# av-savchenko/HSE_FaceRec_tf

Measured on AMD Instinct MI355X. Metric: faces/sec embedding-extract (MobileNet-192, bs=256), higher is better.
Workload: dtype f32

## Files before the change

### hse_facerec_tf_amd/_lib.py

```python
from __future__ import annotations

import ctypes
import os
from ctypes import POINTER, c_char_p, c_float, c_int, c_longlong, c_size_t, c_void_p

_HERE = os.path.dirname(os.path.abspath(__file__))
LIB_PATH = os.path.join(_HERE, os.environ.get("HSEFR_LIB", "libhsefr.so"))

OK, ERR_INVALID, ERR_UNSUPPORTED, ERR_HIP, ERR_NOMEM, ERR_SHAPE = 0, -1, -2, -3, -4, -5

_lib = None

_fp = c_void_p
SIGNATURES = {
    "hsefr_version": (c_int, []),
    "hsefr_last_error_string": (c_char_p, []),
    "hsefr_engine_set_graph_batch": (c_int, [c_void_p, c_int]),
    "hsefr_engine_graph_launches": (c_longlong, [c_void_p]),
    "hsefr_engine_create": (c_int, [c_void_p, c_size_t, c_int, POINTER(c_void_p)]),
    "hsefr_plan_validate": (c_int, [c_void_p, c_size_t]),
    "hsefr_plan_describe": (c_int, [c_void_p, c_size_t, c_int, c_char_p, c_size_t]),
    "hsefr_engine_workspace_bytes": (c_size_t, [c_void_p]),
    "hsefr_engine_max_batch": (c_int, [c_void_p]),
    "hsefr_engine_forward": (c_int, [c_void_p, _fp, c_int, _fp, _fp, _fp, c_void_p]),
    "hsefr_engine_buffer": (c_void_p, [c_void_p, c_int]),
    "hsefr_engine_copy_buffer": (c_int, [c_void_p, c_int, _fp, c_size_t, c_void_p]),
    "hsefr_engine_set_profiling": (c_int, [c_void_p, c_int]),
    "hsefr_engine_profiled_calls": (c_longlong, [c_void_p]),
    "hsefr_engine_op_times_ms": (c_int, [c_void_p, c_int, POINTER(c_float), c_int]),
    "hsefr_engine_destroy": (c_int, [c_void_p]),
    "hsefr_conv_c3_bias_act": (c_int, [_fp, _fp, _fp, _fp] + [c_int] * 12 + [c_void_p]),
    "hsefr_dwconv3x3_bn_relu6": (c_int, [_fp, _fp, _fp, _fp, _fp] + [c_int] * 10 + [c_void_p]),
    "hsefr_dwconv3x3_bn_relu6_split": (c_int, [_fp, _fp, _fp, _fp, _fp] + [c_int] * 11 + [c_void_p]),
    "hsefr_pwconv1x1_presplit_gap": (c_int, [_fp, c_void_p, _fp, _fp, _fp, c_longlong, c_int, c_int, c_int, c_int, c_void_p]),
    "hsefr_pwconv1x1_presplit_dw": (c_int, [_fp, c_void_p, _fp, _fp, _fp, _fp, c_longlong] + [c_int] * 7 + [c_void_p]),
    "hsefr_pwconv1x1_presplit": (c_int, [_fp, c_void_p, _fp, _fp, _fp, c_longlong, c_int, c_int, c_int, c_void_p]),
    "hsefr_pwconv1x1_bias_relu6": (c_int, [_fp, _fp, _fp, _fp, c_longlong, c_int, c_int, c_int, c_void_p]),
    "hsefr_stem2_fused": (c_int, [_fp] * 6 + [c_void_p] + [_fp] * 6 + [c_int] * 13 + [c_void_p]),
    "hsefr_stem3_fused": (c_int, [_fp, c_void_p] + [_fp] * 5 + [c_void_p] + [_fp] * 7 + [c_int] * 14 + [c_void_p]),
    "hsefr_stem4_fused": (c_int, [_fp, c_int, c_void_p] + [_fp] * 5 + [c_void_p] + [_fp] * 7 + [c_int] * 6 + [c_void_p]),
    "hsefr_stem5_stream": (c_int, [_fp, c_int, c_void_p] + [_fp] * 5 + [c_void_p] + [_fp] * 7 + [c_int] * 6 + [c_void_p]),
    "hsefr_engine_accepts_u8": (c_int, [c_void_p]),
    "hsefr_engine_forward_u8": (c_int, [c_void_p, _fp, c_int, _fp, _fp, _fp, c_void_p]),
    "hsefr_engine_input_overflow": (c_int, [c_void_p, POINTER(c_int), c_void_p]),
    "hsefr_engine_input_overflow_async": (c_int, [c_void_p, POINTER(c_int), c_void_p]),
    "hsefr_dwpw_f16split": (c_int, [_fp, _fp, _fp, _fp, c_void_p, _fp, _fp, _fp] + [c_int] * 12 + [c_void_p]),
    "hsefr_pwconv1x1_f16split": (c_int, [_fp, c_void_p, _fp, _fp, _fp, c_longlong, c_int, c_int, c_int, c_int, c_void_p]),
    "hsefr_dwpw_fused": (c_int, [_fp] * 7 + [c_int] * 10 + [c_void_p]),
    "hsefr_gap": (c_int, [_fp, _fp, c_int, c_int, c_int, c_void_p]),
    "hsefr_dense": (c_int, [_fp, _fp, _fp, _fp, c_int, c_int, c_int, c_int, c_void_p]),
    "hsefr_softmax": (c_int, [_fp, _fp, c_int, c_int, c_void_p]),
    "hsefr_heads_fused": (c_int, [_fp] * 11 + [c_int] * 3 + [c_void_p]),
    "hsefr_conv_bf16": (c_int, [_fp, _fp, _fp, _fp, _fp, _fp] + [c_int] * 13 + [c_void_p]),
    "hsefr_conv1x1_proj_bf16": (c_int, [_fp] * 9 + [c_int] * 10 + [c_void_p]),
    "hsefr_conv1x1_sres_bf16": (c_int, [_fp] * 6 + [c_int] * 9 + [c_void_p]),
    "hsefr_conv1x1_pair_bf16": (c_int, [_fp] * 14 + [c_longlong] + [c_int] * 6 + [c_void_p]),
    "hsefr_conv1x1_pair_sub2_bf16": (c_int, [_fp] * 14 + [c_int] * 9 + [c_void_p]),
    "hsefr_stem7x7_bf16": (c_int, [_fp, _fp, _fp, _fp, _fp] + [c_int] * 6 + [c_void_p]),
    "hsefr_stem7x7_pool_bf16": (c_int, [_fp, c_void_p, _fp, _fp, c_void_p] + [c_int] * 7 + [c_void_p]),
    "hsefr_maxpool3x3s2_bf16": (c_int, [_fp, _fp] + [c_int] * 8 + [c_void_p]),
    "hsefr_gap_bf16": (c_int, [_fp, _fp, c_int, c_int, c_int, c_void_p]),
    "hsefr_preprocess_pil_u8": (c_int, [_fp, _fp, _fp] + [c_int] * 5 + [_fp, _fp, _fp, c_int, _fp, _fp, _fp, c_int, c_int,
                                        POINTER(ctypes.c_double), c_void_p]),
    "hsefr_preprocess_cv_u8": (c_int, [_fp, _fp] + [c_int] * 5 + [_fp] * 6 + [c_int, POINTER(ctypes.c_double), c_void_p]),
    "hsefr_l2_normalize": (c_int, [_fp, _fp, c_int, c_int, c_void_p]),
    "hsefr_conv2d_direct": (c_int, [_fp] * 5 + [c_int] * 12 + [c_void_p]),
    "hsefr_conv2d_f32": (c_int, [_fp] * 6 + [c_int] * 13 + [c_void_p]),
    "hsefr_conv2d_f32_mfma": (c_int, [_fp] * 6 + [c_int] * 13 + [c_void_p]),
    "hsefr_maxpool_f32": (c_int, [_fp, _fp] + [c_int] * 10 + [c_void_p]),
    "hsefr_mtcnn_pyramid_level": (c_int, [_fp, _fp, c_int, c_int, c_int, c_int, c_void_p]),
    "hsefr_mtcnn_post_capacity": (c_int, []),
    "hsefr_mtcnn_stage1_level": (c_int, [_fp, _fp, c_int, c_int, ctypes.c_double, ctypes.c_float, _fp, _fp, c_void_p]),
    "hsefr_mtcnn_stage1_finish": (c_int, [_fp, _fp, _fp, _fp, c_int, c_int, c_void_p]),
    "hsefr_mtcnn_stage_finish": (c_int, [c_int, _fp, c_int, _fp, _fp, _fp, ctypes.c_float, _fp, _fp, _fp, _fp, c_int, c_int, c_void_p]),
    "hsefr_mtcnn_nms": (c_int, [_fp, c_int, ctypes.c_double, c_int, _fp, _fp, c_void_p]),
    "hsefr_mtcnn_crops": (c_int, [_fp, _fp, _fp, c_int, c_int, c_int, c_int, c_void_p]),
    "hsefr_pairwise_dist": (c_int, [_fp, _fp, c_int, c_int, c_int, _fp, c_void_p]),
    "hsefr_single_linkage": (c_int, [_fp, c_int, c_int, _fp, _fp, _fp, _fp, _fp, _fp, c_void_p]),
    "hsefr_hier_linkage": (c_int, [_fp, c_int, c_int, _fp, _fp, _fp, c_int, _fp, _fp, _fp, _fp, c_void_p]),
    "hsefr_dbscan": (c_int, [_fp, c_int, c_int, _fp, _fp, _fp, ctypes.c_double, c_int, _fp, _fp, c_void_p]),
    "hsefr_rank_order": (c_int, [_fp, c_int, c_int, _fp, _fp, _fp, ctypes.c_double, ctypes.c_double, _fp, POINTER(c_int), c_void_p]),
    "hsefr_rank_order_sweep": (c_int, [_fp, c_int, c_int, _fp, _fp, _fp, POINTER(ctypes.c_double), c_int, _fp, POINTER(c_int), c_void_p]),
    "hsefr_flat_cuts": (c_int, [_fp, _fp, c_int, _fp, c_int, _fp, c_void_p]),
    "hsefr_partition_scores": (c_int, [_fp, _fp, c_int, c_int, _fp, _fp, c_void_p]),
    "hsefr_nn1": (c_int, [_fp, _fp, c_int, c_int, c_int, _fp, _fp, c_void_p]),
    "hsefr_knn": (c_int, [_fp, _fp, c_int, c_int, c_int, c_int, _fp, _fp, _fp, _fp, c_void_p]),
    "hsefr_nn1_fallbacks": (c_longlong, []),
    "hsefr_pca_fit": (c_int, [_fp, c_int, c_int, c_int, c_int, _fp, _fp, _fp, _fp, c_void_p]),
    "hsefr_pca_transform": (c_int, [_fp, c_int, c_int, c_int, _fp, _fp, _fp, c_int, c_void_p]),
    "hsefr_linear_svm_fit": (c_int, [_fp, c_int, c_int, _fp, c_int, ctypes.c_double, ctypes.c_double, c_int, _fp, _fp, _fp, c_void_p]),
    "hsefr_linear_svm_decision": (c_int, [_fp, c_int, c_int, _fp, _fp, c_int, _fp, c_void_p]),
    "hsefr_linear_svm_predict": (c_int, [_fp, c_int, c_int, _fp, c_void_p]),
    "hsefr_rbf_svm_gamma_scale": (c_int, [_fp, c_int, c_int, c_int, _fp, c_void_p]),
    "hsefr_rbf_svm_fit": (c_int, [_fp, c_int, c_int, _fp, c_int, ctypes.c_double, ctypes.c_double, ctypes.c_double, c_int, _fp, _fp, _fp,
                                  c_void_p]),
    "hsefr_rbf_svm_decision": (c_int, [_fp, c_int, _fp, c_int, c_int, _fp, c_int, ctypes.c_double, _fp, _fp, _fp, c_void_p]),
    "hsefr_rbf_svm_predict": (c_int, [_fp, c_int, _fp, c_int, c_int, _fp, c_int, ctypes.c_double, _fp, _fp, _fp, _fp, c_void_p]),
}

DEV_SIGNATURES = {
    "hsefr_debug_set": (c_int, [c_char_p, c_int]),
    "hsefr_debug_read_stamps": (c_int, [c_int, c_void_p, ctypes.c_size_t]),
    "hsefr_debug_clock_probe": (c_int, [_fp, c_int, c_int, c_void_p]),
    "hsefr_debug_copy": (c_int, [_fp, _fp, c_size_t, c_void_p]),
    "hsefr_stem_fused": (c_int, [_fp] * 6 + [c_void_p, _fp, _fp, _fp] + [c_int] * 9 + [c_void_p]),
}


class HsefrError(RuntimeError):
    pass


def lib() -> ctypes.CDLL:
    global _lib
    if _lib is None:
        import torch
        if not os.path.exists(LIB_PATH):
            raise ImportError("%s is missing: build it with `python -c 'import __graft_entry__ as g; g.build()'` "
                              "(hipcc --offload-arch=gfx950). There is no CPU fallback." % LIB_PATH)
        L = ctypes.CDLL(LIB_PATH)
        for name, (res, args) in SIGNATURES.items():
            fn = getattr(L, name)
            fn.restype = res
            fn.argtypes = args
        for name, (res, args) in DEV_SIGNATURES.items():
            if hasattr(L, name):
                fn = getattr(L, name)
                fn.restype = res
                fn.argtypes = args
# ... 75 lines not shown
```

### hse_facerec_tf_amd/csrc/common.h

```cpp
#pragma once
#include <hip/hip_runtime.h>
#include <stdarg.h>
#include <stdio.h>

#include "../../include/hsefr.h"
#ifdef HSEFR_DEV
#include "hsefr_dev.h"
#endif

namespace hsefr {

void set_error(const char* fmt, ...);

#define HSEFR_HIP_CHECK(expr)                                                          \
    do {                                                                               \
        hipError_t _e = (expr);                                                        \
        if (_e != hipSuccess) {                                                        \
            ::hsefr::set_error("%s failed: %s (%s:%d)", #expr, hipGetErrorString(_e),  \
                               __FILE__, __LINE__);                                    \
            return HSEFR_ERR_HIP;                                                      \
        }                                                                              \
    } while (0)

#define HSEFR_REQUIRE(cond, code, ...)     \
// ... 167 lines not shown
bool conv3x3_win_bf16_supported(long long n, int h, int w, int c, int cout);
int launch_conv3x3_win_bf16(const void* x, const void* wt, const float* scale, const float* shift, const void* res, void* y, int n, int h,
                            int w, int c, int cout, int act, hipStream_t s);
bool conv3x3_w2_forced();
bool conv3x3_w2_bf16_supported(long long n, int h, int w, int c, int cout);
bool conv3x3_w2_bf16_preferred(int h, int w, int cout);
int launch_conv3x3_w2_bf16(const void* x, const void* wt, const float* scale, const float* shift, const void* res, void* y, int n, int h,
                           int w, int c, int cout, int act, hipStream_t s);
bool conv1x1_w4_forced();
bool conv1x1_w4_bf16_supported(long long n, int h, int w, int c, int oh, int ow, int cout, int stride);
bool conv1x1_w4_bf16_preferred(long long pixels, int c, int cout, bool has_res);
bool conv1x1_w4_proj_preferred(long long pixels, int c, int c2, int cout);
int launch_conv1x1_w4_proj_bf16(const void* x, const void* wt, const float* scale, const float* shift, const void* x2, const void* wt2,
                                const float* scale2, const float* shift2, void* y, int n, int oh, int ow, int c, int cout, int c2, int stride2,
                                int h2, int w2, int act, hipStream_t s);
int launch_conv1x1_w4_bf16(const void* x, const void* wt, const float* scale, const float* shift, const void* res, void* y, int n, int h,
                           int w, int c, int oh, int ow, int cout, int stride, int act, hipStream_t s);
bool conv1x1_pair_bf16_shape_supported(int c, int cout1, int cout2, int c2);
bool conv1x1_pair_bf16_supported(long long pixels, int c, int cout1, int cout2, int c2);
int launch_conv1x1_pair_bf16(const void* x, const void* w1, const float* scale1, const float* shift1, const void* res, const void* x2,
                             const void* wp, const float* scale_p, const float* shift_p, void* y1, const void* w2, const float* scale2,
                             const float* shift2, void* y2, long long pixels, int c, int cout1, int cout2, int c2, int act1, int act2,
                             hipStream_t s, int y1_stride = 1, int h = 0, int w = 0);
bool conv_dma_forced();
bool conv_dma_bf16_supported(long long n, int h, int w, int c, int oh, int ow, int cout, int kh, int kw);
int launch_conv_dma_bf16(const void* x, const void* wt, const float* scale, const float* shift, const void* res, void* y, int n, int h,
                         int w, int c, int oh, int ow, int cout, int kh, int kw, int stride, int pad_t, int pad_l, int act, hipStream_t s);
int launch_stem7x7_pool_bf16(const float* x, const void* wt, const float* scale, const float* shift, void* y, int n, int h, int w,
                             int ph, int pw, int pool_pad_t, int pool_pad_l, hipStream_t s, const void* wfrag = nullptr);
bool stem7s_stream_supported(long long n, int h, int w, int ph, int pw);
int launch_stem7s_stream(const float* x, const void* wt, const float* scale, const float* shift, void* y, int n, int h, int w, int ph, int pw,
                         int pool_pad_t, int pool_pad_l, hipStream_t s, const void* wfrag = nullptr);
constexpr size_t STEM7S_WFRAG_BYTES = 4 * 7 * 64 * 16;
int stem7s_reorder_weights(const void* wt, void* wfrag, hipStream_t s);
int launch_maxpool3x3s2_bf16(const void* x, void* y, int n, int h, int w, int c, int oh, int ow, int pad_t, int pad_l,
                             hipStream_t s);
int launch_gap_bf16(const void* x, float* y, int n, int hw, int c, hipStream_t s);

int launch_pil_resize(const unsigned char* in, unsigned char* tmp, float* out, int n, int H, int W, int oh, int ow, const int* xmin,
                      const int* xcnt, const int* xcoef, int xk, const int* ymin, const int* ycnt, const int* ycoef, int yk,
                      int mode, const double* mean, hipStream_t s);
int launch_cv_resize(const unsigned char* in, float* out, int n, int H, int W, int oh, int ow, const int* x0, const int* x1,
                     const int* wx1, const int* y0, const int* y1, const int* wy1, int mode, const double* mean, hipStream_t s);

int launch_area_level(const unsigned char* src, float* dst, int sh, int sw, int dh, int dw, hipStream_t s);
int launch_area_crops(const unsigned char* src, const int* boxes, float* dst, int sh, int sw, int n, int size, hipStream_t s);
int launch_pairwise_dist(const float* x, const float* y, int n, int m, int d, float* out, hipStream_t s);
struct DistSource {
    const float* x;
    int n, d;
    const float* born;
    const float* year;
    const double* dense;
};
int launch_single_linkage(const DistSource& src, int* edge_a, int* edge_b, double* edge_h, hipStream_t s);
int launch_dbscan(const DistSource& src, double eps, int min_samples, int* labels, unsigned char* core, hipStream_t s);
int launch_rank_order(const DistSource& src, const double* thresholds, int pairs, int* labels, int* iterations, hipStream_t s);
int launch_hier_linkage(const DistSource& src, int method, int* merge_a, int* merge_b, double* merge_h, int* merge_round, hipStream_t s);
int launch_flat_cuts(const int* order, const double* gaps, int n, const double* thresholds, int rows, int* labels, hipStream_t s);
int launch_partition_scores(const int* y_true, const int* labels, int n, int rows, long long* counts, double* stats, hipStream_t s);

bool dwpw_fused_supported(int c, int cout, int stride, int act_dw, int act_pw);
int launch_dwpw_fused(const float* x, const float* wd, const float* dscale, const float* dshift, const float* wp_t,
                      const float* pshift, float* y, int n, int h, int w, int c, int stride, int pad_t, int pad_l, int oh,
                      int ow, int cout, int act_dw, int act_pw, hipStream_t s);

int launch_conv2d_direct(const float* x, const float* w, const float* bias, const float* alpha, float* y, int n, int h, int wd, int c,
                         int oh, int ow, int cout, int kh, int kw, int stride, int pad_t, int pad_l, hipStream_t s);
int launch_conv_f32_mfma(const float* x, const float* w, const float* scale, const float* shift, const float* res, float* y, int n, int h,
                         int wd, int c, int oh, int ow, int cout, int kh, int kw, int stride, int pad_t, int pad_l, int act, hipStream_t s,
                         int res_stride = 0, int res_h = 0, int res_w = 0);
bool conv_f32_mfma_supported(int c, int cout);
int launch_conv2d_f32(const float* x, const float* w, const float* scale, const float* shift, const float* res, float* y, int n, int h,
                      int wd, int c, int oh, int ow, int cout, int kh, int kw, int stride, int pad_t, int pad_l, int act, hipStream_t s);
int launch_maxpool_f32(const float* x, float* y, int n, int h, int w, int c, int oh, int ow, int k, int stride, int pad_t, int pad_l,
                       hipStream_t s);

int launch_dwpw_f16s(const float* x, const float* wd, const float* dscale, const float* dshift, const void* wsplit,
                     const float* descale, const float* pshift, float* y, int n, int h, int w, int c, int stride, int pad_t,
                     int pad_l, int oh, int ow, int cout, int a_log2, int act, hipStream_t s);
bool dwpw_f16s_supported(int c, int cout, int stride);
bool dwpw_s2_covered(int c, int cout, int stride);
bool dwpw_s2_off();
int launch_stem_fused(const float* x, const float* cw, const float* cshift, const float* wd, const float* dscale,
                      const float* dshift, const void* wsplit, const float* descale, const float* pshift, float* y, int n,
                      int h, int w, int cpad_t, int cpad_l, int oh, int ow, int a_log2, int act, hipStream_t s);
int launch_stem2_fused(const float* x, const float* cw, const float* cshift, const float* wd1, const float* d1scale,
                       const float* d1shift, const void* wsplit, const float* descale, const float* pshift, const float* wd2,
                       const float* d2scale, const float* d2shift, float* y, int n, int h, int w, int cpad_t, int cpad_l,
                       int h1, int w1, int pad_t2, int pad_l2, int oh2, int ow2, int a_log2, int act, hipStream_t s);
int launch_stem3_fused(const float* x, const void* cw_split, const float* cdescale, const float* cshift, const float* wd1,
                       const float* d1scale, const float* d1shift, const void* wsplit, const float* descale, const float* pshift,
                       const float* wd2, const float* d2scale, const float* d2shift, float* y, int* overflow, int n, int h, int w,
                       int cpad_t, int cpad_l, int h1, int w1, int pad_t2, int pad_l2, int oh2, int ow2, int in_log2, int a_log2,
                       int act, hipStream_t s);
bool stem3_fused_supported(int cin, int c1, int c2, int conv_stride, int dw1_stride, int dw2_stride, int kh, int kw);
int launch_stem4_fused(const void* x, int x_is_u8, const void* cw4, const float* cdescale, const float* cshift, const float* wd1,
                       const float* d1scale, const float* d1shift, const void* wsplit, const float* descale, const float* pshift,
                       const float* wd2, const float* d2scale, const float* d2shift, float* y, int* overflow, int n, int h, int w,
                       int in_log2, int a_log2, int act, hipStream_t s);
bool stem4_fused_supported(int cin, int c1, int c2, int conv_stride, int dw1_stride, int dw2_stride, int kh, int kw, int h, int w);
int launch_stem5_stream(const void* x, int x_is_u8, const void* cw4, const float* cdescale, const float* cshift, const float* wd1,
                        const float* d1scale, const float* d1shift, const void* wsplit, const float* descale, const float* pshift,
                        const float* wd2, const float* d2scale, const float* d2shift, float* y, int* overflow, int n, int h, int w,
                        int in_log2, int a_log2, int act, hipStream_t s);
bool stem5_stream_supported(int cin, int c1, int c2, int conv_stride, int dw1_stride, int dw2_stride, int kh, int kw, int h, int w);
bool stem2_fused_supported(int cin, int c1, int c2, int conv_stride, int dw1_stride, int dw2_stride, int kh, int kw);
bool stem_fused_supported(int cin, int cmid, int cout, int conv_stride, int dw_stride, int kh, int kw);
int read_pws_stamps(void* host_out, size_t bytes);
int read_stem_stamps(void* host_out, size_t bytes);
#ifdef HSEFR_STEM_STAMPS
unsigned long long* stamp_buffer(hipStream_t s);
#define STEM_STAMP(i) do { const unsigned long long _t = __builtin_amdgcn_s_memtime(); st[i] += _t - tprev; tprev = _t; } while (0)
#define STEM_STAMP_DECL unsigned long long st[8] = {0, 0, 0, 0, 0, 0, 0, 0}; unsigned long long tprev = __builtin_amdgcn_s_memtime(); \
    const unsigned long long tstart = tprev; unsigned npatch = 0
#define STEM_STAMP_COUNT ++npatch
#define STEM_STAMP_FLUSH(buf, lane, wave) do { if ((lane) == 0 && (buf) && blockIdx.x < 512) { unsigned long long* o = (buf) + (blockIdx.x * 4 + (wave)) * 10; \
    for (int i_ = 0; i_ < 8; ++i_) o[i_] = st[i_]; o[8] = __builtin_amdgcn_s_memtime() - tstart; o[9] = npatch; } } while (0)
#else
#define STEM_STAMP(i) do { } while (0)
#define STEM_STAMP_DECL do { } while (0)
#define STEM_STAMP_COUNT do { } while (0)
#define STEM_STAMP_FLUSH(buf, lane, wave) do { } while (0)
#endif
#ifdef HSEFR_DEV
int read_c11_stamps(void* host_out, size_t bytes);
int read_w4_stamps(void* host_out, size_t bytes);
int read_s7_stamps(void* host_out, size_t bytes);
int read_w2_stamps(void* host_out, size_t bytes);
int read_w3_stamps(void* host_out, size_t bytes);
int read_cd_stamps(void* host_out, size_t bytes);
int read_ps_stamps(void* host_out, size_t bytes);
int launch_clock_probe(unsigned long long* out, int blocks, int iters, hipStream_t s);
int launch_copy(const void* src, void* dst, size_t bytes, hipStream_t s);
#endif

}
```

### hse_facerec_tf_amd/csrc/engine.hip

```cpp
#include <math.h>
#include <string.h>

#include <cxxabi.h>
#include <dlfcn.h>
#include <elf.h>

#include <map>
#include <new>
#include <string>
#include <vector>

#include "common.h"

namespace hsefr {

static thread_local char g_err[512] = "";

void set_error(const char* fmt, ...) {
    va_list ap;
    va_start(ap, fmt);
    vsnprintf(g_err, sizeof(g_err), fmt, ap);
    va_end(ap);
}

// ... 185 lines not shown
                break;
            case HSEFR_OP_PWCONV_PS_GAP:
                HSEFR_REQUIRE(pwconv_ps_gap_supported(0, o.cin, o.cout, o.h * o.w) && o.oh == 1 && o.ow == 1, HSEFR_ERR_UNSUPPORTED,
                              "plan op %u: fused pointwise + global pool on a %dx%d map not covered (33 .. 288 pixels)", i, o.h, o.w);
                if (!need(o.w_off, ci * co * 4, "split rows") || !need(o.scale_off, co * 4, "descale") || !need(o.shift_off, co * 4, "shift"))
                    return HSEFR_ERR_INVALID;
                HSEFR_REQUIRE(o.aux > 0 && o.aux <= 24, HSEFR_ERR_INVALID, "plan op %u: a_log2 out of range (reserved %d)", i, o.aux);
                break;
            case HSEFR_OP_PWCONV_PS_DW:
                HSEFR_REQUIRE(pwconv_ps_dw_supported(0, o.cin, o.cout, o.w, o.h * o.w, o.stride) && o.oh * o.stride == o.h && o.ow * o.stride == o.w &&
                                  (o.stride == 1 ? (o.pad_t == 1 && o.pad_l == 1) : (o.pad_t == 0 && o.pad_l == 0)),
                              HSEFR_ERR_UNSUPPORTED, "plan op %u: fused pointwise + depthwise (stride %d) on a %dx%d map not covered", i, o.stride, o.h, o.w);
                if (!need(o.w_off, ci * co * 4, "split rows") || !need(o.scale_off, co * 4, "descale") || !need(o.shift_off, co * 4, "shift") ||
                    !need(o.w2_off, 11 * co * 4, "depthwise constants"))
                    return HSEFR_ERR_INVALID;
                {
                    const PsDwAux a = ps_dw_aux(o.aux);
                    HSEFR_REQUIRE(a.a_log2 > 0 && a.a_log2 <= 24 && a.out_log2 >= 1 && a.out_log2 <= 12,
                                  HSEFR_ERR_INVALID, "plan op %u: a_log2 / out_log2 out of range (reserved %d)", i, o.aux);
                }
                break;
            case HSEFR_OP_PWCONV_PS:
                HSEFR_REQUIRE(pwconv_ps_supported(0, o.cin, o.cout), HSEFR_ERR_UNSUPPORTED,
                              "plan op %u: pre-split pointwise cin=%d cout=%d not covered", i, o.cin, o.cout);
                [[fallthrough]];
            case HSEFR_OP_PWCONV_F16S:
                if (!need(o.w_off, ci * co * 4, "split rows") || !need(o.scale_off, co * 4, "descale") || !need(o.shift_off, co * 4, "shift"))
                    return HSEFR_ERR_INVALID;
                HSEFR_REQUIRE(o.w_off != HSEFR_NO_OFFSET && o.scale_off != HSEFR_NO_OFFSET && o.shift_off != HSEFR_NO_OFFSET &&
                                  o.aux > 0 && o.aux <= 24,
                              HSEFR_ERR_INVALID, "plan op %u: split-f16 pointwise needs split rows, descale, shift and a_log2 in (0, 24]", i);
                break;
            case HSEFR_OP_STEM3_F16S: {
                const StemAux a = stem_aux(o.aux);
                HSEFR_REQUIRE(stem3_fused_supported(o.cin, 32, o.cout, o.stride, 1, 2, o.kh, stem_kw(o.kw).k) && a.a_log2 > 0 && a.a_log2 <= 12 &&
                                  a.in_log2 >= -8 && a.in_log2 <= 14 &&
                                  o.w_off != HSEFR_NO_OFFSET && o.w2_off != HSEFR_NO_OFFSET && o.shift2_off != HSEFR_NO_OFFSET &&
                                  o.w_off + HSEFR_STEM_PACK_STEM3_END * 4 <= h.blob_bytes && o.w2_off + 64 * 128 <= h.blob_bytes &&
                                  o.shift2_off + 128 * 4 <= h.blob_bytes && o.in_buf == HSEFR_BUF_INPUT,
                              HSEFR_ERR_UNSUPPORTED, "plan op %u: bounded fused stem cin=%d cout=%d stride=%d not covered", i, o.cin, o.cout, o.stride);
                break;
            }
            case HSEFR_OP_STEM2_F16S:
                HSEFR_REQUIRE(stem2_fused_supported(o.cin, 32, o.cout, o.stride, 1, 2, o.kh, stem_kw(o.kw).k) && o.aux > 0 && o.aux <= 12 &&
                                  o.w_off != HSEFR_NO_OFFSET && o.w2_off != HSEFR_NO_OFFSET && o.shift2_off != HSEFR_NO_OFFSET &&
                                  o.w_off + HSEFR_STEM_PACK_STEM2_END * 4 <= h.blob_bytes && o.in_buf == HSEFR_BUF_INPUT,
                              HSEFR_ERR_UNSUPPORTED, "plan op %u: fused stem+dw2 cin=%d cout=%d stride=%d not covered", i, o.cin, o.cout, o.stride);
                break;
            case HSEFR_OP_STEM_F16S:
#ifndef HSEFR_DEV
                set_error("plan op %u: HSEFR_OP_STEM_F16S (round 1's fused stem) runs on development builds of the library only", i);
                return HSEFR_ERR_UNSUPPORTED;
#else
                HSEFR_REQUIRE(stem_fused_supported(o.cin, 32, o.cout, o.stride, 1, o.kh, o.kw) && o.aux > 0 && o.aux <= 12 &&
                                  o.w_off != HSEFR_NO_OFFSET && o.w2_off != HSEFR_NO_OFFSET && o.shift2_off != HSEFR_NO_OFFSET &&
                                  o.w_off + HSEFR_STEM_PACK_DW2 * 4 <= h.blob_bytes && o.in_buf == HSEFR_BUF_INPUT,
                              HSEFR_ERR_UNSUPPORTED, "plan op %u: fused stem cin=%d cout=%d stride=%d not covered", i, o.cin, o.cout, o.stride);
                break;
#endif
            case HSEFR_OP_DWPW_F16S:
                if (!need(o.w_off, 9 * ci * 4, "depthwise kernel") || !need(o.scale_off, ci * 4, "scale") || !need(o.shift_off, ci * 4, "shift") ||
                    !need(o.w2_off, ci * co * 4, "split rows") || !need(o.shift2_off, 2 * co * 4, "descale | shift"))
                    return HSEFR_ERR_INVALID;
                HSEFR_REQUIRE(dwpw_f16s_supported(o.cin, o.cout, o.stride) && o.aux > 0 && o.aux <= 12 &&
                                  o.w_off != HSEFR_NO_OFFSET && o.scale_off != HSEFR_NO_OFFSET && o.shift_off != HSEFR_NO_OFFSET &&
                                  o.w2_off != HSEFR_NO_OFFSET && o.shift2_off != HSEFR_NO_OFFSET,
                              HSEFR_ERR_UNSUPPORTED, "plan op %u: split-f16 fused block cin=%d cout=%d stride=%d a_log2=%d not covered",
                              i, o.cin, o.cout, o.stride, o.aux);
                break;
            case HSEFR_OP_DWPW_F32:
                if (!need(o.w_off, 9 * ci * 4, "depthwise kernel") || !need(o.scale_off, ci * 4, "scale") || !need(o.shift_off, ci * 4, "shift") ||
                    !need(o.w2_off, ci * co * 4, "pointwise kernel") || !need(o.shift2_off, co * 4, "pointwise shift"))
                    return HSEFR_ERR_INVALID;
                HSEFR_REQUIRE(dwpw_fused_supported(o.cin, o.cout, o.stride, HSEFR_ACT_RELU6, (int)o.act), HSEFR_ERR_UNSUPPORTED,
                              "plan op %u: fused depthwise-pointwise block cin=%d cout=%d not covered", i, o.cin, o.cout);
                break;
            default:
                set_error("plan op %u: unknown kind %u", i, o.kind);
                return HSEFR_ERR_UNSUPPORTED;
        }
    }
    for (uint32_t i = 0; i < h.n_ops; ++i) {
        const hsefr_plan_op& o = ops[i];
        HSEFR_REQUIRE((o.flags & ~(HSEFR_OPF_PAIR_NEXT | HSEFR_OPF_HEADS | HSEFR_OPF_OUT_SUB2 | HSEFR_OPF_DWPW_NEXT)) == 0, HSEFR_ERR_INVALID,
                      "plan op %u: unknown flags 0x%x", i, o.flags);
        HSEFR_REQUIRE(!(o.flags & HSEFR_OPF_OUT_SUB2) || (o.flags & HSEFR_OPF_PAIR_NEXT), HSEFR_ERR_INVALID, "plan op %u: OUT_SUB2 without PAIR_NEXT", i);
        if (o.flags & HSEFR_OPF_PAIR_NEXT) {
            HSEFR_REQUIRE(i + 1 < h.n_ops, HSEFR_ERR_INVALID, "plan op %u: PAIR_NEXT on the last op", i);
            const hsefr_plan_op& b = ops[i + 1];
            const bool proj = o.w2_off != HSEFR_NO_OFFSET;
            const Geometry g = geometry(o.aux);
            const int c2 = proj ? g.c2 : 0;
            const bool sub2 = (o.flags & HSEFR_OPF_OUT_SUB2) != 0;
            HSEFR_REQUIRE(o.kind == HSEFR_OP_CONV_BF16 && b.kind == HSEFR_OP_CONV_BF16 && o.kh == 1 && o.kw == 1 && o.stride == 1 && o.pad_t == 0 &&
                              o.pad_l == 0 && (sub2 ? (o.oh == (o.h + 1) / 2 && o.ow == (o.w + 1) / 2 && o.h > 1 && o.w > 1) : (o.oh == o.h && o.ow == o.w)) &&
                              b.kh == 1 && b.kw == 1 && b.stride == 1 && b.pad_t == 0 && b.pad_l == 0 &&
                              b.h == o.h && b.w == o.w && b.oh == b.h && b.ow == b.w && b.cin == o.cout && b.in_buf == o.out_buf &&
                              b.res_buf == HSEFR_BUF_NONE && b.w2_off == HSEFR_NO_OFFSET && b.flags == 0 && o.res_buf >= 0 &&
                              (!proj || (g.stride2 == 1 && g.h2 == o.h && g.w2 == o.w)),
                          HSEFR_ERR_INVALID, "plan op %u: PAIR_NEXT needs two 1x1 stride-1 bf16 convolutions at the same pixels, the first with a residual "
                          "or a same-pixel projected shortcut, the second reading the first", i);
            HSEFR_REQUIRE(b.out_buf != o.in_buf && b.out_buf != o.res_buf && b.out_buf != o.out_buf, HSEFR_ERR_INVALID,
                          "plan op %u: PAIR_NEXT: the second output (buffer %d) aliases an operand of the first", i, b.out_buf);
            HSEFR_REQUIRE(conv1x1_pair_bf16_shape_supported(o.cin, o.cout, b.cout, c2), HSEFR_ERR_UNSUPPORTED,
                          "plan op %u: PAIR_NEXT %d -> %d -> %d (projection from %d) not covered", i, o.cin, o.cout, b.cout, c2);
        }
        if (o.flags & HSEFR_OPF_DWPW_NEXT) {
            HSEFR_REQUIRE(o.flags == HSEFR_OPF_DWPW_NEXT && i + 1 < h.n_ops, HSEFR_ERR_INVALID, "plan op %u: DWPW_NEXT on the last op or beside another flag", i);
            const hsefr_plan_op& b = ops[i + 1];
            HSEFR_REQUIRE(o.kind == HSEFR_OP_DWCONV3X3 && o.stride == 2 && o.act == HSEFR_ACT_RELU6 && o.aux == 0 && o.cout == o.cin &&
                              b.kind == HSEFR_OP_PWCONV_F16S && b.in_buf == o.out_buf && b.flags == 0 && b.h == o.oh && b.w == o.ow && b.oh == b.h &&
                              b.ow == b.w && b.cin == o.cin && b.aux > 0 && b.aux <= 12,
                          HSEFR_ERR_INVALID, "plan op %u: DWPW_NEXT needs a stride-2 depthwise 3x3 with ReLU6 and fp32 output, and behind it a split-f16 "
                          "pointwise op without flags that reads it at the same pixels (a_log2 in [1, 12])", i);
            HSEFR_REQUIRE(dwpw_s2_covered(o.cin, b.cout, o.stride), HSEFR_ERR_INVALID, "plan op %u: DWPW_NEXT %d -> %d channels not covered (128 -> 256)", i,
                          o.cin, b.cout);
            HSEFR_REQUIRE(b.out_buf != o.out_buf, HSEFR_ERR_INVALID, "plan op %u: DWPW_NEXT: the second output (buffer %d) aliases the depthwise tensor", i,
                          b.out_buf);
            HSEFR_REQUIRE(b.out_buf != o.in_buf || (uint64_t)bufs[o.in_buf].elems_per_image * bufs[o.in_buf].elem_bytes ==
                                                       (uint64_t)bufs[o.out_buf].elems_per_image * bufs[o.out_buf].elem_bytes,
                          HSEFR_ERR_INVALID, "plan op %u: DWPW_NEXT: buffers %d and %d exchange roles and must have one size", i, o.in_buf, o.out_buf);
            for (uint32_t k = i + 2; k < h.n_ops; ++k) {
                HSEFR_REQUIRE(ops[k].in_buf != o.out_buf && ops[k].res_buf != o.out_buf, HSEFR_ERR_INVALID,
                              "plan op %u: DWPW_NEXT: op %u also reads the depthwise tensor (buffer %d)", i, k, o.out_buf);
                if (ops[k].out_buf == o.out_buf) break;
            }
            for (int sl = 0; sl < HSEFR_N_OUTPUT_SLOTS; ++sl)
                HSEFR_REQUIRE(h.out_buffer[sl] != o.out_buf && (b.out_buf != o.in_buf || h.out_buffer[sl] != o.in_buf), HSEFR_ERR_INVALID,
                              "plan op %u: DWPW_NEXT: the depthwise tensor (or the buffer it exchanges roles with) is output slot %d", i, sl);
        }
        if (o.flags & HSEFR_OPF_HEADS) {
            HSEFR_REQUIRE(i + 3 < h.n_ops, HSEFR_ERR_INVALID, "plan op %u: HEADS needs three ops behind it", i);
            const hsefr_plan_op &a = ops[i + 1], &sm = ops[i + 2], &g = ops[i + 3];
            HSEFR_REQUIRE(o.kind == HSEFR_OP_DENSE && o.act == HSEFR_ACT_RELU && o.cout == 256 && o.cin > 0 && o.cin % 256 == 0 && o.cin <= 2048 &&
                              o.shift_off != HSEFR_NO_OFFSET && a.kind == HSEFR_OP_DENSE && a.act == HSEFR_ACT_NONE && a.cin == 256 && a.cout >= 1 &&
                              a.cout <= 128 && a.in_buf == o.out_buf && a.shift_off != HSEFR_NO_OFFSET && sm.kind == HSEFR_OP_SOFTMAX &&
                              sm.in_buf == a.out_buf && sm.cout == a.cout && g.kind == HSEFR_OP_DENSE && g.act == HSEFR_ACT_SIGMOID && g.cin == 256 &&
                              g.cout == 1 && g.in_buf == o.out_buf && g.shift_off != HSEFR_NO_OFFSET && a.flags == 0 && sm.flags == 0 && g.flags == 0,
                          HSEFR_ERR_INVALID, "plan op %u: HEADS needs DENSE k -> 256 + ReLU, DENSE 256 -> a (<= 128) + bias, SOFTMAX, DENSE 256 -> 1 + sigmoid", i);
            const int outs[4] = {o.out_buf, a.out_buf, sm.out_buf, g.out_buf};
            for (int x = 0; x < 4; ++x) {
                HSEFR_REQUIRE(outs[x] != o.in_buf, HSEFR_ERR_INVALID, "plan op %u: HEADS: an output aliases the pooled features", i);
                for (int y = x + 1; y < 4; ++y)
                    HSEFR_REQUIRE(outs[x] != outs[y], HSEFR_ERR_INVALID, "plan op %u: HEADS: two of the four tensors share buffer %d", i, outs[x]);
            }
        }
    }
    for (int s = 0; s < HSEFR_N_OUTPUT_SLOTS; ++s) {
        HSEFR_REQUIRE(h.out_buffer[s] == HSEFR_BUF_NONE || (h.out_buffer[s] >= 0 && h.out_buffer[s] < (int)h.n_buffers),
                      HSEFR_ERR_INVALID, "plan: output slot %d names buffer %d", s, h.out_buffer[s]);
        if (h.out_buffer[s] == HSEFR_BUF_NONE) continue;
        const int b = h.out_buffer[s];
        uint32_t producers = 0;
        for (uint32_t i = 0; i < h.n_ops; ++i) producers += (ops[i].out_buf == b);
        HSEFR_REQUIRE(producers == 1, HSEFR_ERR_INVALID, "plan: output slot %d: buffer %d has %u producing ops (must be exactly 1)", s, b,
                      producers);
        HSEFR_REQUIRE((uint64_t)bufs[b].elems_per_image * bufs[b].elem_bytes == (uint64_t)h.out_elems[s] * 4, HSEFR_ERR_INVALID,
                      "plan: output slot %d: buffer %d holds %llu x %u bytes per image, the slot declares %u fp32 elements", s, b,
                      (unsigned long long)bufs[b].elems_per_image, (unsigned)bufs[b].elem_bytes, h.out_elems[s]);
    }
    return HSEFR_OK;
}

namespace hsefr {
#ifdef HSEFR_STEM_STAMPS
static unsigned long long* g_stamp_buf = nullptr;
unsigned long long* stamp_buffer(hipStream_t s) {
    if (!g_stamp_buf && hipMalloc((void**)&g_stamp_buf, 512 * 4 * 10 * 8) != hipSuccess) return nullptr;
    (void)hipMemsetAsync(g_stamp_buf, 0, 512 * 4 * 10 * 8, s);
    return g_stamp_buf;
}
int read_stem_stamps(void* host_out, size_t bytes) {
    HSEFR_REQUIRE(g_stamp_buf && bytes <= 512 * 4 * 10 * 8, HSEFR_ERR_INVALID, "read_stem_stamps: nothing recorded / too many bytes");
    HSEFR_HIP_CHECK(hipMemcpy(host_out, g_stamp_buf, bytes, hipMemcpyDeviceToHost));
    return HSEFR_OK;
}
#else
int read_stem_stamps(void* host_out, size_t bytes) {
    (void)host_out; (void)bytes;
    set_error("read_stem_stamps: library built without -DHSEFR_STEM_STAMPS");
    return HSEFR_ERR_UNSUPPORTED;
}
#endif
static thread_local std::string* g_route_sink = nullptr;
bool route_probe() { return g_route_sink != nullptr; }
static const std::map<uintptr_t, std::string>& stub_names() {
    static const std::map<uintptr_t, std::string> table = [] {
        std::map<uintptr_t, std::string> m;
        Dl_info info;
        if (!dladdr(reinterpret_cast<const void*>(&stub_names), &info) || !info.dli_fname) return m;
        FILE* f = fopen(info.dli_fname, "rb");
        if (!f) return m;
        std::vector<unsigned char> img;
        fseek(f, 0, SEEK_END);
        const long sz = ftell(f);
        fseek(f, 0, SEEK_SET);
        if (sz > 0) { img.resize((size_t)sz); if (fread(img.data(), 1, img.size(), f) != img.size()) img.clear(); }
        fclose(f);
        if (img.size() < sizeof(Elf64_Ehdr)) return m;
        const Elf64_Ehdr* eh = reinterpret_cast<const Elf64_Ehdr*>(img.data());
        if (memcmp(eh->e_ident, ELFMAG, SELFMAG) != 0 || eh->e_shentsize != sizeof(Elf64_Shdr) ||
            eh->e_shoff + (uint64_t)eh->e_shnum * sizeof(Elf64_Shdr) > img.size()) return m;
        const Elf64_Shdr* sh = reinterpret_cast<const Elf64_Shdr*>(img.data() + eh->e_shoff);
        for (int i = 0; i < eh->e_shnum; ++i) {
            if (sh[i].sh_type != SHT_SYMTAB || sh[i].sh_link >= eh->e_shnum) continue;
            const Elf64_Shdr& st = sh[sh[i].sh_link];
            if (sh[i].sh_offset + sh[i].sh_size > img.size() || st.sh_offset + st.sh_size > img.size()) continue;
            const Elf64_Sym* sym = reinterpret_cast<const Elf64_Sym*>(img.data() + sh[i].sh_offset);
            const char* str = reinterpret_cast<const char*>(img.data() + st.sh_offset);
            for (size_t k = 0; k < sh[i].sh_size / sizeof(Elf64_Sym); ++k) {
                if (ELF64_ST_TYPE(sym[k].st_info) != STT_OBJECT || sym[k].st_name >= st.sh_size) continue;
                const char* nm = str + sym[k].st_name;
// ... 182 lines not shown

int hsefr_engine_copy_buffer(hsefr_engine* e, int buffer, void* d_dst, size_t bytes, hsefr_stream_t stream) {
    HSEFR_REQUIRE(e && d_dst, HSEFR_ERR_INVALID, "copy_buffer: null argument");
    HSEFR_REQUIRE(buffer >= 0 && buffer < (int)e->d_bufs.size(), HSEFR_ERR_INVALID, "copy_buffer: buffer %d", buffer);
    const size_t cap = (size_t)e->bufs[buffer].elems_per_image * e->bufs[buffer].elem_bytes * e->max_batch;
    HSEFR_REQUIRE(bytes <= cap, HSEFR_ERR_SHAPE, "copy_buffer: %zu bytes exceed buffer %d (%zu)", bytes, buffer, cap);
    HSEFR_HIP_CHECK(hipMemcpyAsync(d_dst, e->d_bufs[buffer], bytes, hipMemcpyDeviceToDevice, (hipStream_t)stream));
    return HSEFR_OK;
}

int hsefr_engine_set_profiling(hsefr_engine* e, int depth) {
    HSEFR_REQUIRE(e && depth >= 0, HSEFR_ERR_INVALID, "set_profiling: bad argument");
    for (auto ev : e->events) (void)hipEventDestroy(ev);
    e->events.clear();
    e->prof_depth = 0;
    e->prof_calls = 0;
    if (depth > 0) {
        e->events.resize((size_t)depth * (e->ops.size() + 1));
        for (auto& ev : e->events) HSEFR_HIP_CHECK(hipEventCreate(&ev));
        e->prof_depth = depth;
    }
    return HSEFR_OK;
}

long long hsefr_engine_profiled_calls(const hsefr_engine* e) { return e ? e->prof_calls : 0; }

int hsefr_engine_op_times_ms(hsefr_engine* e, int slot, float* ms, int n_ops) {
    HSEFR_REQUIRE(e && ms, HSEFR_ERR_INVALID, "op_times: null argument");
    HSEFR_REQUIRE(e->prof_depth > 0 && slot >= 0 && slot < e->prof_depth && slot < e->prof_calls, HSEFR_ERR_INVALID,
                  "op_times: slot %d has no profiled forward (depth %d, calls %lld)", slot, e->prof_depth, e->prof_calls);
    HSEFR_REQUIRE(n_ops == (int)e->ops.size(), HSEFR_ERR_INVALID, "op_times: expected %zu ops", e->ops.size());
    hipEvent_t* ev = e->events.data() + (size_t)slot * (e->ops.size() + 1);
    HSEFR_HIP_CHECK(hipEventSynchronize(ev[n_ops]));
    for (int i = 0; i < n_ops; ++i) HSEFR_HIP_CHECK(hipEventElapsedTime(&ms[i], ev[i], ev[i + 1]));
    return HSEFR_OK;
}

struct Operands {
    const void *w, *w2;
    const float *scale, *shift, *shift2;
};
static Operands operands(const hsefr_engine* e, const hsefr_plan_op& o) {
    return {blob_ptr(e, o.w_off), blob_ptr(e, o.w2_off), (const float*)blob_ptr(e, o.scale_off), (const float*)blob_ptr(e, o.shift_off),
            (const float*)blob_ptr(e, o.shift2_off)};
}

static int launch_op(hsefr_engine* e, size_t i, std::vector<void*>& tab, const void* d_input, int n, const std::vector<char>& needed, hipStream_t s,
                     bool input_u8, bool every_tensor, size_t& covered) {
    const hsefr_plan_op& o = e->ops[i];
    const Operands p = operands(e, o);
    const void* in = buf_ptr(tab, o.in_buf, d_input);
    void* out = buf_ptr(tab, o.out_buf, d_input);
    const long long pixels = (long long)n * o.h * o.w;
    covered = 0;
    const bool sub2 = (o.flags & HSEFR_OPF_OUT_SUB2) != 0;
    const Geometry g = geometry(o.aux);
    const bool proj = o.w2_off != HSEFR_NO_OFFSET;
    const int c2 = proj ? g.c2 : 0;
    const bool pair_ok = (o.flags & HSEFR_OPF_PAIR_NEXT) && needed[i + 1] &&
                         conv1x1_pair_bf16_supported(pixels, o.cin, o.cout, e->ops[i + 1].cout, c2);
    HSEFR_REQUIRE(!sub2 || pair_ok, HSEFR_ERR_UNSUPPORTED, "forward: op %zu stores its output at every second pixel (OUT_SUB2) and cannot run without the pair launch", i);
    if (pair_ok) {
        const hsefr_plan_op& b = e->ops[i + 1];
        const Operands pb = operands(e, b);
        covered = 1;
        return launch_conv1x1_pair_bf16(in, p.w, p.scale, p.shift, proj ? nullptr : tab[o.res_buf], proj ? tab[o.res_buf] : nullptr, proj ? p.w2 : nullptr,
                                        proj ? p.shift2 : nullptr, proj ? p.shift2 + o.cout : nullptr, out, pb.w, pb.scale, pb.shift, tab[b.out_buf],
                                        pixels, o.cin, o.cout, b.cout, c2, o.act, b.act, s, sub2 ? 2 : 1, o.h, o.w);
    }
    if ((o.flags & HSEFR_OPF_HEADS) && !g_heads_off && needed[i + 1] && needed[i + 2] && needed[i + 3]) {
        const hsefr_plan_op &a = e->ops[i + 1], &sm = e->ops[i + 2], &gd = e->ops[i + 3];
        const Operands pa = operands(e, a), pg = operands(e, gd);
        covered = 3;
        return launch_heads_fused((const float*)in, (const float*)p.w, p.shift, (const float*)pa.w, pa.shift, (const float*)pg.w, pg.shift, (float*)out,
                                  (float*)tab[a.out_buf], (float*)tab[sm.out_buf], (float*)tab[gd.out_buf], n, o.cin, a.cout, s);
    }
    if ((o.flags & HSEFR_OPF_DWPW_NEXT) && !every_tensor && !dwpw_s2_off() && needed[i + 1]) {
        const hsefr_plan_op& b = e->ops[i + 1];
        const Operands pb = operands(e, b);
        if (b.out_buf == o.in_buf) std::swap(tab[o.in_buf], tab[o.out_buf]);
        covered = 1;
        return launch_dwpw_f16s((const float*)in, (const float*)p.w, p.scale, p.shift, pb.w, pb.scale, pb.shift, (float*)tab[b.out_buf], n, o.h, o.w,
                                o.cin, o.stride, o.pad_t, o.pad_l, o.oh, o.ow, b.cout, b.aux, b.act, s);
    }
    const void* res = o.res_buf >= 0 ? tab[o.res_buf] : nullptr;
    switch (o.kind) {
        case HSEFR_OP_CONV_C3:
            return launch_conv_c3((const float*)in, (const float*)p.w, p.shift, (float*)out, n, o.h, o.w, o.kh, o.kw, o.stride, o.pad_t, o.pad_l, o.oh, o.ow,
                                  o.cout, o.act, s);
        case HSEFR_OP_DWCONV3X3:
            if (o.aux > 0)
                return launch_dwconv3x3_split((const float*)in, (const float*)p.w, p.scale, p.shift, out, n, o.h, o.w, o.cin, o.stride, o.pad_t, o.pad_l,
                                              o.oh, o.ow, o.act, o.aux, s);
            return launch_dwconv3x3((const float*)in, (const float*)p.w, p.scale, p.shift, (float*)out, n, o.h, o.w, o.cin, o.stride, o.pad_t, o.pad_l, o.oh,
                                    o.ow, o.act, s);
        case HSEFR_OP_PWCONV_PS_GAP:
            return launch_pwconv_ps_gap(in, p.w, p.scale, p.shift, (float*)out, pixels, o.cin, o.cout, o.act, o.h * o.w, s);
        case HSEFR_OP_PWCONV_PS_DW:
            return launch_pwconv_ps_dw(in, p.w, p.scale, p.shift, (const float*)p.w2, out, pixels, o.cin, o.cout, o.act, o.w, o.h * o.w, o.stride,
                                       ps_dw_aux(o.aux).out_log2, s);
        case HSEFR_OP_PWCONV_PS:
            return launch_pwconv_ps(in, p.w, p.scale, p.shift, (float*)out, pixels, o.cin, o.cout, o.act, s);
        case HSEFR_OP_PWCONV_F32:
            return launch_pwconv_f32((const float*)in, (const float*)p.w, p.shift, (float*)out, pixels, o.cin, o.cout, o.act, s);
        case HSEFR_OP_PWCONV_F16S:
            return launch_pwconv_f16s((const float*)in, p.w, p.scale, p.shift, (float*)out, pixels, o.cin, o.cout, o.aux, o.act, s);
        case HSEFR_OP_GAP:
            return launch_gap((const float*)in, (float*)out, n, o.h * o.w, o.cin, s);
        case HSEFR_OP_DENSE:
            return launch_dense((const float*)in, (const float*)p.w, p.shift, (float*)out, n, o.cin, o.cout, o.act, s);
        case HSEFR_OP_SOFTMAX:
            return launch_softmax((const float*)in, (float*)out, n, o.cout, s);
        case HSEFR_OP_CONV_BF16:
            if (proj)
                return launch_conv1x1_proj_bf16(in, p.w, p.scale, p.shift, tab[o.res_buf], p.w2, p.shift2, p.shift2 + o.cout, out, n, o.oh, o.ow, o.cin,
                                                o.cout, g.c2, g.stride2, g.h2, g.w2, o.act, s);
            if (o.res_buf >= 0 && o.aux != 0)
                return launch_conv1x1_sres_bf16(in, p.w, p.scale, p.shift, res, out, n, o.oh, o.ow, o.cin, o.cout, g.stride2, g.h2, g.w2, o.act, s);
            return launch_conv_bf16(in, p.w, p.scale, p.shift, res, out, n, o.h, o.w, o.cin, o.oh, o.ow, o.cout, o.kh, o.kw, o.stride, o.pad_t, o.pad_l,
                                    o.act, s);
        case HSEFR_OP_CONV_F32:
            if (conv_f32_mfma_supported(o.cin, o.cout))
                return launch_conv_f32_mfma((const float*)in, (const float*)p.w, p.scale, p.shift, (const float*)res, (float*)out, n, o.h, o.w, o.cin, o.oh,
                                            o.ow, o.cout, o.kh, o.kw, o.stride, o.pad_t, o.pad_l, o.act, s, o.res_buf >= 0 ? g.stride2 : 0, g.h2, g.w2);
            return launch_conv2d_f32((const float*)in, (const float*)p.w, p.scale, p.shift, (const float*)res, (float*)out, n, o.h, o.w, o.cin, o.oh, o.ow,
                                     o.cout, o.kh, o.kw, o.stride, o.pad_t, o.pad_l, o.act, s);
        case HSEFR_OP_MAXPOOL_F32:
            return launch_maxpool_f32((const float*)in, (float*)out, n, o.h, o.w, o.cin, o.oh, o.ow, o.kh, o.stride, o.pad_t, o.pad_l, s);
        case HSEFR_OP_STEM7X7_BF16:
            return launch_stem7x7_bf16((const float*)in, p.w, p.scale, p.shift, out, n, o.h, o.w, o.oh, o.ow, o.act, s);
        case HSEFR_OP_STEM7X7_POOL_BF16:
            return launch_stem7x7_pool_bf16((const float*)in, p.w, p.scale, p.shift, out, n, o.h, o.w, o.oh, o.ow, pool_pads(o.aux).t, pool_pads(o.aux).l, s,
                                            i < e->d_derived.size() ? e->d_derived[i] : nullptr);
        case HSEFR_OP_MAXPOOL_BF16:
            return launch_maxpool3x3s2_bf16(in, out, n, o.h, o.w, o.cin, o.oh, o.ow, o.pad_t, o.pad_l, s);
        case HSEFR_OP_GAP_BF16:
            return launch_gap_bf16(in, (float*)out, n, o.h * o.w, o.cin, s);
        case HSEFR_OP_DWPW_F32:
            return launch_dwpw_fused((const float*)in, (const float*)p.w, p.scale, p.shift, (const float*)p.w2, p.shift2, (float*)out, n, o.h, o.w, o.cin,
                                     o.stride, o.pad_t, o.pad_l, o.oh, o.ow, o.cout, HSEFR_ACT_RELU6, o.act, s);
        case HSEFR_OP_STEM3_F16S: {
            const StemPack k = stem_pack(e, o);
            const StemAux a = stem_aux(o.aux);
            const StemKw kw = stem_kw(o.kw);
            if (input_u8)
                return (g_stem5 ? launch_stem5_stream : launch_stem4_fused)(in, 1, k.conv4_u8, k.u8_descale, k.u8_shift, k.dw1, k.dw1_scale, k.dw1_shift, p.w2,
                                                                          k.descale, k.pshift, k.dw2, k.dw2_scale, k.dw2_shift, (float*)out, nullptr, n, o.h,
                                                                          o.w, 0, a.a_log2, o.act, s);
            if (g_stem4 && stem4_route(o))
                return (g_stem5 ? launch_stem5_stream : launch_stem4_fused)(in, 0, k.conv4, k.conv_descale, k.conv_shift, k.dw1, k.dw1_scale, k.dw1_shift, p.w2,
                                                                          k.descale, k.pshift, k.dw2, k.dw2_scale, k.dw2_shift, (float*)out, e->d_overflow, n,
                                                                          o.h, o.w, a.in_log2, a.a_log2, o.act, s);
            return launch_stem3_fused((const float*)in, k.conv_split, k.conv_descale, k.conv_shift, k.dw1, k.dw1_scale, k.dw1_shift, p.w2, k.descale, k.pshift,
                                      k.dw2, k.dw2_scale, k.dw2_shift, (float*)out, e->d_overflow, n, o.h, o.w, o.pad_t, o.pad_l, (o.h + 1) / 2, (o.w + 1) / 2,
                                      kw.pad_t2, kw.pad_l2, o.oh, o.ow, a.in_log2, a.a_log2, o.act, s);
        }
        case HSEFR_OP_STEM2_F16S: {
            const StemPack k = stem_pack(e, o);
            const StemKw kw = stem_kw(o.kw);
            return launch_stem2_fused((const float*)in, k.conv, k.conv_shift, k.dw1, k.dw1_scale, k.dw1_shift, p.w2, k.descale, k.pshift, k.dw2, k.dw2_scale,
                                      k.dw2_shift, (float*)out, n, o.h, o.w, o.pad_t, o.pad_l, (o.h + 1) / 2, (o.w + 1) / 2, kw.pad_t2, kw.pad_l2, o.oh, o.ow,
                                      o.aux, o.act, s);
        }
#ifdef HSEFR_DEV
        case HSEFR_OP_STEM_F16S: {
            const StemPack k = stem_pack(e, o);
// ... 246 lines not shown
    return launch_pwconv_ps_dw(x_split, w_split, descale, shift, dw_consts, y_split, m, k, cout, act, map_w, map_hw, dw_stride, out_log2,
                               (hipStream_t)stream);
}

int hsefr_pwconv1x1_presplit(const void* x_split, const void* w_split, const float* descale, const float* shift, float* y,
                             long long m, int k, int cout, int act, hsefr_stream_t stream) {
    HSEFR_REQUIRE(m == 0 || (x_split && w_split && descale && shift && y), HSEFR_ERR_INVALID, "pwconv_presplit: null pointer");
    return launch_pwconv_ps(x_split, w_split, descale, shift, y, m, k, cout, act, (hipStream_t)stream);
}

int hsefr_pwconv1x1_bias_relu6(const float* x, const float* wgt_t, const float* shift, float* y, long long m, int k,
                               int cout, int act, hsefr_stream_t stream) {
    HSEFR_REQUIRE(m == 0 || (x && wgt_t && shift && y), HSEFR_ERR_INVALID, "pwconv: null pointer");
    return launch_pwconv_f32(x, wgt_t, shift, y, m, k, cout, act, (hipStream_t)stream);
}

int hsefr_pwconv1x1_f16split(const float* x, const void* w_split, const float* descale, const float* shift, float* y,
                             long long m, int k, int cout, int a_log2, int act, hsefr_stream_t stream) {
    HSEFR_REQUIRE(m == 0 || (x && w_split && descale && shift && y), HSEFR_ERR_INVALID, "pwconv_f16split: null pointer");
    return launch_pwconv_f16s(x, w_split, descale, shift, y, m, k, cout, a_log2, act, (hipStream_t)stream);
}

int hsefr_stem2_fused(const float* x, const float* conv_w, const float* conv_shift, const float* wd1, const float* d1scale,
                      const float* d1shift, const void* w_split, const float* descale, const float* pshift, const float* wd2,
                      const float* d2scale, const float* d2shift, float* y, int n, int h, int w, int cpad_t, int cpad_l,
                      int h1, int w1, int pad_t2, int pad_l2, int oh2, int ow2, int a_log2, int act, hsefr_stream_t stream) {
    HSEFR_REQUIRE(n == 0 || (x && conv_w && conv_shift && wd1 && d1scale && d1shift && w_split && descale && pshift && wd2 &&
                             d2scale && d2shift && y), HSEFR_ERR_INVALID, "stem2_fused: null pointer");
    return launch_stem2_fused(x, conv_w, conv_shift, wd1, d1scale, d1shift, w_split, descale, pshift, wd2, d2scale, d2shift, y, n,
                              h, w, cpad_t, cpad_l, h1, w1, pad_t2, pad_l2, oh2, ow2, a_log2, act, (hipStream_t)stream);
}

int hsefr_stem3_fused(const float* x, const void* cw_split, const float* cdescale, const float* conv_shift, const float* wd1,
                      const float* d1scale, const float* d1shift, const void* w_split, const float* descale, const float* pshift,
                      const float* wd2, const float* d2scale, const float* d2shift, float* y, int* d_overflow, int n, int h, int w,
                      int cpad_t, int cpad_l, int h1, int w1, int pad_t2, int pad_l2, int oh2, int ow2, int in_log2, int a_log2,
                      int act, hsefr_stream_t stream) {
    HSEFR_REQUIRE(n == 0 || (x && cw_split && cdescale && conv_shift && wd1 && d1scale && d1shift && w_split && descale && pshift && wd2 &&
                             d2scale && d2shift && y), HSEFR_ERR_INVALID, "stem3_fused: null pointer");
    return launch_stem3_fused(x, cw_split, cdescale, conv_shift, wd1, d1scale, d1shift, w_split, descale, pshift, wd2, d2scale, d2shift, y,
                              d_overflow, n, h, w, cpad_t, cpad_l, h1, w1, pad_t2, pad_l2, oh2, ow2, in_log2, a_log2, act, (hipStream_t)stream);
}

int hsefr_stem4_fused(const void* x, int x_is_u8, const void* cw4, const float* cdescale, const float* conv_shift, const float* wd1,
                      const float* d1scale, const float* d1shift, const void* w_split, const float* descale, const float* pshift,
                      const float* wd2, const float* d2scale, const float* d2shift, float* y, int* d_overflow, int n, int h, int w,
                      int in_log2, int a_log2, int act, hsefr_stream_t stream) {
    HSEFR_REQUIRE(n == 0 || (x && cw4 && cdescale && conv_shift && wd1 && d1scale && d1shift && w_split && descale && pshift && wd2 &&
                             d2scale && d2shift && y), HSEFR_ERR_INVALID, "stem4_fused: null pointer");
    return launch_stem4_fused(x, x_is_u8, cw4, cdescale, conv_shift, wd1, d1scale, d1shift, w_split, descale, pshift, wd2, d2scale, d2shift, y,
                              d_overflow, n, h, w, in_log2, a_log2, act, (hipStream_t)stream);
}

int hsefr_stem5_stream(const void* x, int x_is_u8, const void* cw4, const float* cdescale, const float* conv_shift, const float* wd1,
                       const float* d1scale, const float* d1shift, const void* w_split, const float* descale, const float* pshift,
                       const float* wd2, const float* d2scale, const float* d2shift, float* y, int* d_overflow, int n, int h, int w,
                       int in_log2, int a_log2, int act, hsefr_stream_t stream) {
    HSEFR_REQUIRE(n == 0 || (x && cw4 && cdescale && conv_shift && wd1 && d1scale && d1shift && w_split && descale && pshift && wd2 &&
                             d2scale && d2shift && y), HSEFR_ERR_INVALID, "stem5_stream: null pointer");
    return launch_stem5_stream(x, x_is_u8, cw4, cdescale, conv_shift, wd1, d1scale, d1shift, w_split, descale, pshift, wd2, d2scale, d2shift, y,
                               d_overflow, n, h, w, in_log2, a_log2, act, (hipStream_t)stream);
}

#ifdef HSEFR_DEV
int hsefr_stem_fused(const float* x, const float* conv_w, const float* conv_shift, const float* wd, const float* dscale,
                     const float* dshift, const void* w_split, const float* descale, const float* pshift, float* y, int n,
                     int h, int w, int cpad_t, int cpad_l, int oh, int ow, int a_log2, int act, hsefr_stream_t stream) {
    HSEFR_REQUIRE(n == 0 || (x && conv_w && conv_shift && wd && dscale && dshift && w_split && descale && pshift && y),
                  HSEFR_ERR_INVALID, "stem_fused: null pointer");
    return launch_stem_fused(x, conv_w, conv_shift, wd, dscale, dshift, w_split, descale, pshift, y, n, h, w, cpad_t, cpad_l,
                             oh, ow, a_log2, act, (hipStream_t)stream);
}
#endif

int hsefr_dwpw_f16split(const float* x, const float* wd, const float* dscale, const float* dshift, const void* w_split,
                        const float* descale, const float* pshift, float* y, int n, int h, int w, int c, int stride,
                        int pad_t, int pad_l, int oh, int ow, int cout, int a_log2, int act, hsefr_stream_t stream) {
    HSEFR_REQUIRE(n == 0 || (x && wd && dscale && dshift && w_split && descale && pshift && y), HSEFR_ERR_INVALID,
                  "dwpw_f16split: null pointer");
    return launch_dwpw_f16s(x, wd, dscale, dshift, w_split, descale, pshift, y, n, h, w, c, stride, pad_t, pad_l, oh, ow, cout,
                            a_log2, act, (hipStream_t)stream);
}

int hsefr_dwpw_fused(const float* x, const float* wd, const float* dscale, const float* dshift, const float* wp_t,
                     const float* pshift, float* y, int n, int h, int w, int c, int stride, int pad_t, int pad_l, int oh,
                     int ow, int cout, hsefr_stream_t stream) {
    HSEFR_REQUIRE(n == 0 || (x && wd && dscale && dshift && wp_t && pshift && y), HSEFR_ERR_INVALID, "dwpw_fused: null pointer");
    return launch_dwpw_fused(x, wd, dscale, dshift, wp_t, pshift, y, n, h, w, c, stride, pad_t, pad_l, oh, ow, cout,
                             HSEFR_ACT_RELU6, HSEFR_ACT_RELU6, (hipStream_t)stream);
}

int hsefr_gap(const float* x, float* y, int n, int hw, int c, hsefr_stream_t stream) {
    HSEFR_REQUIRE(n == 0 || (x && y), HSEFR_ERR_INVALID, "gap: null pointer");
    return launch_gap(x, y, n, hw, c, (hipStream_t)stream);
}

int hsefr_dense(const float* x, const float* wgt, const float* bias, float* y, int n, int k, int cout, int act,
                hsefr_stream_t stream) {
    HSEFR_REQUIRE(n == 0 || (x && wgt && y), HSEFR_ERR_INVALID, "dense: null pointer");
    return launch_dense(x, wgt, bias, y, n, k, cout, act, (hipStream_t)stream);
}

int hsefr_heads_fused(const float* x, const float* w1, const float* b1, const float* wa, const float* ba, const float* wg, const float* bg,
                      float* hidden, float* logits, float* age_probs, float* gender, int n, int k, int a, hsefr_stream_t stream) {
    HSEFR_REQUIRE(n == 0 || (x && w1 && b1 && wa && ba && wg && bg && hidden && logits && age_probs && gender), HSEFR_ERR_INVALID,
                  "heads_fused: null pointer");
    return launch_heads_fused(x, w1, b1, wa, ba, wg, bg, hidden, logits, age_probs, gender, n, k, a, (hipStream_t)stream);
}

int hsefr_softmax(const float* x, float* y, int n, int c, hsefr_stream_t stream) {
    HSEFR_REQUIRE(n == 0 || (x && y), HSEFR_ERR_INVALID, "softmax: null pointer");
    return launch_softmax(x, y, n, c, (hipStream_t)stream);
}

int hsefr_conv_bf16(const void* x, const void* wgt_t, const float* scale, const float* shift, const void* res, void* y,
                    int n, int h, int w, int c, int oh, int ow, int cout, int kh, int kw, int stride, int pad_t,
                    int pad_l, int act, hsefr_stream_t stream) {
    HSEFR_REQUIRE(n == 0 || (x && wgt_t && scale && shift && y), HSEFR_ERR_INVALID, "conv_bf16: null pointer");
    return launch_conv_bf16(x, wgt_t, scale, shift, res, y, n, h, w, c, oh, ow, cout, kh, kw, stride, pad_t, pad_l, act,
                            (hipStream_t)stream);
}

int hsefr_conv1x1_proj_bf16(const void* x, const void* wgt_t, const float* scale, const float* shift, const void* x2, const void* wgt2_t,
                            const float* scale2, const float* shift2, void* y, int n, int oh, int ow, int c, int cout, int c2, int stride2,
                            int h2, int w2, int act, hsefr_stream_t stream) {
    HSEFR_REQUIRE(n == 0 || (x && wgt_t && scale && shift && x2 && wgt2_t && scale2 && shift2 && y), HSEFR_ERR_INVALID, "conv1x1_proj_bf16: null pointer");
    return launch_conv1x1_proj_bf16(x, wgt_t, scale, shift, x2, wgt2_t, scale2, shift2, y, n, oh, ow, c, cout, c2, stride2, h2, w2, act,
                                    (hipStream_t)stream);
}

int hsefr_conv1x1_sres_bf16(const void* x, const void* wgt_t, const float* scale, const float* shift, const void* res, void* y, int n, int oh,
                            int ow, int c, int cout, int res_stride, int h2, int w2, int act, hsefr_stream_t stream) {
    HSEFR_REQUIRE(n == 0 || (x && wgt_t && scale && shift && res && y), HSEFR_ERR_INVALID, "conv1x1_sres_bf16: null pointer");
    return launch_conv1x1_sres_bf16(x, wgt_t, scale, shift, res, y, n, oh, ow, c, cout, res_stride, h2, w2, act, (hipStream_t)stream);
}

int hsefr_conv1x1_pair_bf16(const void* x, const void* w1_t, const float* scale1, const float* shift1, const void* res, const void* x2,
                            const void* wp_t, const float* scale_p, const float* shift_p, void* y1, const void* w2_t, const float* scale2,
                            const float* shift2, void* y2, long long pixels, int c, int cout1, int cout2, int c2, int act1, int act2,
                            hsefr_stream_t stream) {
    HSEFR_REQUIRE(pixels >= 0, HSEFR_ERR_INVALID, "conv1x1_pair_bf16: pixels=%lld", pixels);
    if (pixels == 0) return HSEFR_OK;
    HSEFR_REQUIRE(x && w1_t && scale1 && shift1 && y1 && w2_t && scale2 && shift2 && y2 && (c2 == 0 ? res != nullptr : (x2 && wp_t && scale_p && shift_p)),
                  HSEFR_ERR_INVALID, "conv1x1_pair_bf16: null pointer");
    return launch_conv1x1_pair_bf16(x, w1_t, scale1, shift1, c2 == 0 ? res : nullptr, x2, wp_t, scale_p, shift_p, y1, w2_t, scale2, shift2, y2, pixels,
                                    c, cout1, cout2, c2, act1, act2, (hipStream_t)stream);
}

int hsefr_conv1x1_pair_sub2_bf16(const void* x, const void* w1_t, const float* scale1, const float* shift1, const void* res, const void* x2,
                                 const void* wp_t, const float* scale_p, const float* shift_p, void* y1, const void* w2_t, const float* scale2,
                                 const float* shift2, void* y2, int n, int h, int w, int c, int cout1, int cout2, int c2, int act1, int act2,
                                 hsefr_stream_t stream) {
    HSEFR_REQUIRE(n >= 0 && h > 1 && w > 1, HSEFR_ERR_INVALID, "conv1x1_pair_sub2_bf16: %d maps of %dx%d", n, h, w);
    if (n == 0) return HSEFR_OK;
    HSEFR_REQUIRE(x && w1_t && scale1 && shift1 && y1 && w2_t && scale2 && shift2 && y2 && (c2 == 0 ? res != nullptr : (x2 && wp_t && scale_p && shift_p)),
                  HSEFR_ERR_INVALID, "conv1x1_pair_sub2_bf16: null pointer");
    return launch_conv1x1_pair_bf16(x, w1_t, scale1, shift1, c2 == 0 ? res : nullptr, x2, wp_t, scale_p, shift_p, y1, w2_t, scale2, shift2, y2,
                                    (long long)n * h * w, c, cout1, cout2, c2, act1, act2, (hipStream_t)stream, 2, h, w);
}

int hsefr_stem7x7_bf16(const float* x, const void* wgt_t, const float* scale, const float* shift, void* y, int n, int h,
                       int w, int oh, int ow, int act, hsefr_stream_t stream) {
    HSEFR_REQUIRE(n == 0 || (x && wgt_t && scale && shift && y), HSEFR_ERR_INVALID, "stem7x7: null pointer");
    return launch_stem7x7_bf16(x, wgt_t, scale, shift, y, n, h, w, oh, ow, act, (hipStream_t)stream);
}

// ... 219 lines not shown
```

### hse_facerec_tf_amd/csrc/fuzz_plan.cc

```cpp
#include <stdint.h>
#include <stdio.h>
#include <stdlib.h>
#include <string.h>

#include <string>
#include <vector>

#include "../../include/hsefr.h"

static uint64_t rng_state = 0x9E3779B97F4A7C15ull;
static uint64_t rnd() {
    rng_state ^= rng_state << 13;
    rng_state ^= rng_state >> 7;
    rng_state ^= rng_state << 17;
    return rng_state;
}

static long long n_ok = 0, n_err = 0, n_silent = 0;
static uint64_t g_hash = 0xcbf29ce484222325ull;
static void fold(int rc) {
    auto mix = [](unsigned char b) { g_hash = (g_hash ^ b) * 0x100000001b3ull; };
    for (int k = 0; k < 4; ++k) mix((unsigned char)((uint32_t)rc >> (8 * k)));
    if (rc != HSEFR_OK)
        for (const char* m = hsefr_last_error_string(); *m; ++m) mix((unsigned char)*m);
}

static void run_one(const void* blob, size_t bytes, const char* what) {
    int rc = hsefr_plan_validate(blob, bytes);
    fold(rc);
    if (rc == HSEFR_OK) {
        ++n_ok;
        static char table[1 << 18];
        const int rd = hsefr_plan_describe(blob, bytes, 4, table, sizeof(table));
        fold(rd);
        if (rd != HSEFR_OK && !hsefr_last_error_string()[0]) { ++n_silent; fprintf(stderr, "no message for status %d (%s, plan_describe)\n", rd, what); }
        hsefr_engine* e = nullptr;
        rc = hsefr_engine_create(blob, bytes, 4, &e);
        if (rc == HSEFR_OK) hsefr_engine_destroy(e);
        else if (!hsefr_last_error_string()[0]) { ++n_silent; fprintf(stderr, "no message for status %d (%s, engine_create)\n", rc, what); }
        return;
    }
    ++n_err;
    if (rc > 0 || rc < HSEFR_ERR_SHAPE || !hsefr_last_error_string()[0]) {
        ++n_silent;
        fprintf(stderr, "status %d without a message / outside hsefr_status (%s)\n", rc, what);
    }
    hsefr_engine* e = nullptr;
    const int rc2 = hsefr_engine_create(blob, bytes, 4, &e);
    if (rc2 == HSEFR_OK) { fprintf(stderr, "engine_create accepted what plan_validate refused (%s)\n", what); abort(); }
}

int main(int argc, char** argv) {
    if (argc < 3) { fprintf(stderr, "usage: fuzz_plan <mutants per seed> <plan file>...\n"); return 2; }
    const long long per_seed = atoll(argv[1]);
    static const int32_t edge32[] = {0, 1, -1, -2, -3, 2, 3, 7, 8, 63, 64, 65, 127, 128, 255, 256, 511, 512, 4095, 4096, 65535, 65536, 0x7fffffff,
                                     (int32_t)0x80000000, (int32_t)0xffff0000, 1 << 20, 1 << 24, 1 << 30};
    static const uint64_t edge64[] = {0ull, 1ull, 15ull, 16ull, 17ull, 0xffffffffull, 0x100000000ull, 0x7fffffffffffffffull, 0x8000000000000000ull,
                                      0xffffffffffffffffull, 0xfffffffffffffff0ull};
    for (int f = 2; f < argc; ++f) {
        FILE* fp = fopen(argv[f], "rb");
        if (!fp) { perror(argv[f]); return 2; }
        fseek(fp, 0, SEEK_END);
        const size_t bytes = (size_t)ftell(fp);
        fseek(fp, 0, SEEK_SET);
        std::vector<unsigned char> seed(bytes);
        if (fread(seed.data(), 1, bytes, fp) != bytes) { fprintf(stderr, "short read\n"); return 2; }
        fclose(fp);
        if (bytes < sizeof(hsefr_plan_header)) { fprintf(stderr, "%s: not a plan\n", argv[f]); return 2; }
        hsefr_plan_header h;
        memcpy(&h, seed.data(), sizeof(h));
        const size_t tables = sizeof(h) + (size_t)h.n_buffers * sizeof(hsefr_plan_buffer) + (size_t)h.n_ops * sizeof(hsefr_plan_op);
        if (hsefr_plan_validate(seed.data(), bytes) != HSEFR_OK) {
            fprintf(stderr, "%s: the seed itself is refused: %s\n", argv[f], hsefr_last_error_string());
            return 1;
        }
        unsigned char* w = (unsigned char*)malloc(bytes);
        memcpy(w, seed.data(), bytes);
        char what[160];
        for (long long it = 0; it < per_seed; ++it) {
            const unsigned mode = (unsigned)(rnd() % 10);
            if (mode == 0) {
                size_t cut = (rnd() & 1) ? (size_t)(rnd() % (tables + 64 < bytes ? tables + 64 : bytes)) : (size_t)(rnd() % bytes);
                unsigned char* t = (unsigned char*)malloc(cut ? cut : 1);
                memcpy(t, seed.data(), cut);
                snprintf(what, sizeof(what), "%s truncated to %zu", argv[f], cut);
                run_one(t, cut, what);
                free(t);
                continue;
            }
            const int nmut = 1 + (int)(rnd() % 3);
            size_t where[3];
            unsigned char saved[3][8];
            size_t len[3];
            for (int m = 0; m < nmut; ++m) {
                size_t off;
                if (mode == 1) {
                    off = (size_t)(rnd() % tables);
                    len[m] = 1;
                    memcpy(saved[m], w + off, 1);
                    w[off] ^= (unsigned char)(1u << (rnd() % 8));
                } else if (mode == 2 && bytes > tables) {
                    off = tables + (size_t)(rnd() % (bytes - tables));
                    len[m] = 1;
                    memcpy(saved[m], w + off, 1);
                    w[off] = (unsigned char)rnd();
                } else if (mode <= 6) {
                    off = (size_t)(rnd() % (tables / 4)) * 4;
                    len[m] = 4;
                    memcpy(saved[m], w + off, 4);
                    const int32_t v = edge32[rnd() % (sizeof(edge32) / sizeof(edge32[0]))];
                    memcpy(w + off, &v, 4);
                } else if (mode <= 8) {
                    off = (size_t)(rnd() % (tables / 8)) * 8;
                    len[m] = 8;
                    memcpy(saved[m], w + off, 8);
                    uint64_t v = edge64[rnd() % (sizeof(edge64) / sizeof(edge64[0]))];
                    if (rnd() & 1) v = h.blob_bytes - 64 + (rnd() % 128);
                    if (rnd() % 4 == 0) v &= ~15ull;
                    memcpy(w + off, &v, 8);
                } else {
                    off = (size_t)(rnd() % (tables / 4)) * 4;
                    len[m] = 4;
                    memcpy(saved[m], w + off, 4);
                    const uint32_t v = (uint32_t)rnd();
                    memcpy(w + off, &v, 4);
                }
                where[m] = off;
            }
            snprintf(what, sizeof(what), "%s mode %u at %zu", argv[f], mode, where[0]);
            run_one(w, bytes, what);
            for (int m = nmut - 1; m >= 0; --m) memcpy(w + where[m], saved[m], len[m]);
        }
        if (memcmp(w, seed.data(), bytes) != 0) { fprintf(stderr, "internal: working copy not restored\n"); return 1; }
        free(w);
    }
    printf("fuzz_plan: %lld mutants still valid, %lld refused, hash %016llx, %lld without a message\n", n_ok, n_err, (unsigned long long)g_hash, n_silent);
    return n_silent ? 1 : 0;
}
// ... 1 lines not shown
```

### hse_facerec_tf_amd/lowering.py

```python
from __future__ import annotations

import struct
from dataclasses import dataclass, field
from typing import Dict, List, Optional, Sequence, Tuple

import numpy as np

from .graphdef import Graph, GraphNode

ACT_NONE, ACT_RELU, ACT_RELU6, ACT_SIGMOID = 0, 1, 2, 3
OP_CONV_C3, OP_DWCONV3X3, OP_PWCONV_F32, OP_GAP, OP_DENSE, OP_SOFTMAX = 1, 2, 3, 4, 5, 6
OP_CONV_BF16, OP_MAXPOOL_BF16, OP_GAP_BF16, OP_STEM7X7_BF16, OP_DWPW_F32 = 7, 8, 9, 10, 11
OP_PWCONV_F16S = 12
OP_DWPW_F16S = 13
OP_STEM_F16S = 14
OP_STEM2_F16S = 15
OP_STEM3_F16S = 17
OP_CONV_F32, OP_MAXPOOL_F32 = 18, 19
OP_STEM7X7_POOL_BF16 = 20
OP_PWDW_PS = 21
OP_PWGAP_PS = 22
OP_PWCONV_PS = 16
_BF16_OUT = (OP_CONV_BF16, OP_MAXPOOL_BF16, OP_STEM7X7_BF16, OP_STEM7X7_POOL_BF16)
OUT_FEATURES, OUT_AGE, OUT_GENDER = 0, 1, 2
BUF_INPUT, BUF_NONE = -1, -2
PLAN_MAGIC = 0x314C505246455348
NO_OFFSET = 0xFFFFFFFFFFFFFFFF

_HEADER = struct.Struct("<QIIIIII3i3IQ")
_BUFFER = struct.Struct("<QII")
_OP = struct.Struct("<II3i3i3i3i2iii5Q")
OPF_PAIR_NEXT, OPF_HEADS, OPF_OUT_SUB2, OPF_DWPW_NEXT = 1, 2, 4, 8
AUX_C2_SHIFT, AUX_C2_BITS, AUX_STRIDE2_SHIFT, AUX_STRIDE2_BITS = 0, 12, 12, 2
AUX_H2_SHIFT, AUX_H2_BITS, AUX_W2_SHIFT, AUX_W2_BITS = 14, 9, 23, 9
AUX_LOG2_BITS, AUX_OUT_LOG2_SHIFT, AUX_IN_LOG2_SHIFT, AUX_IN_LOG2_BIAS, AUX_U8_BIT = 8, 8, 8, 64, 16
AUX_POOL_PAD_L_SHIFT = 4
STEM_KW_PAD_T2_BIT, STEM_KW_PAD_L2_BIT = 4, 5
STEM_PACK_CONV, STEM_PACK_CONV_SHIFT, STEM_PACK_DW1, STEM_PACK_DW1_SCALE, STEM_PACK_DW1_SHIFT = 0, 864, 896, 1184, 1216
STEM_PACK_DW2, STEM_PACK_DW2_SCALE, STEM_PACK_DW2_SHIFT, STEM_PACK_STEM2_END = 1248, 1824, 1888, 1952
STEM_PACK_CONV_SPLIT, STEM_PACK_CONV_DESCALE, STEM_PACK_CONV4, STEM_PACK_CONV4_U8 = 1952, 2976, 3008, 5056
STEM_PACK_U8_SHIFT, STEM_PACK_U8_DESCALE, STEM_PACK_STEM3_END = 7104, 7232, 7264
STEM_SHIFT2_DESCALE, STEM_SHIFT2_SHIFT = 0, 64


PRODUCT_KERNEL_FAMILIES = frozenset({
    "stem5_stream_kernel", "stem4_fused_kernel", "stem3_fused_kernel", "stem2_fused_kernel", "conv3x3_c3_kernel", "conv3x3_c3_mfma_kernel",
    "dwconv3x3_kernel", "pwconv_f32_dma_kernel", "pwconv_f32_kernel", "pwconv_f16s_kernel", "pwconv_ps_kernel", "dwpw_fused_kernel",
    "dwpw_f16s_kernel", "dwpw2_f16s_kernel", "dwpw3_f16s_kernel", "dwpws2_f16s_kernel", "gap_kernel", "dense_kernel", "softmax_kernel", "heads_kernel",
    "stem7s_stream_kernel", "stem7x7_pool_bf16_kernel", "stem7x7_bf16_kernel", "maxpool3x3s2_bf16_kernel", "conv_bf16_kernel", "conv1x1_bf16_kernel",
    "conv1x1_w4_bf16_kernel", "conv1x1_pair_bf16_kernel", "conv3x3_w2_bf16_kernel", "conv_dma_bf16_kernel", "gap_bf16_kernel",
    "conv_f32_mfma_kernel", "conv2d_f32_kernel", "maxpool_f32_kernel"})


class LoweringError(NotImplementedError):
    """The graph uses a construct the engine has no kernel for (analogue of TF's
    'No OpKernel was registered' error)."""


def dequantize_min_first_u8(q: np.ndarray, range_min, range_max) -> np.ndarray:
    lo = np.float32(range_min)
    hi = np.float32(range_max)
    if lo == hi:
        return np.full(q.shape, lo, dtype=np.float32)
    step = np.float32(np.float64(hi - lo) / 255.0)
    lo_snapped = np.float32(np.round(lo / step) * step)
    return q.astype(np.float32) * step + lo_snapped


def tf_same_padding(size: int, k: int, stride: int) -> Tuple[int, int]:
    out = (size + stride - 1) // stride
    total = max((out - 1) * stride + k - size, 0)
    return out, total // 2


F16S_ACT_LOG2_RELU6 = 12


def split_pointwise_weights(w_t: np.ndarray, a_log2: int = F16S_ACT_LOG2_RELU6) -> Tuple[np.ndarray, np.ndarray]:
    w = np.ascontiguousarray(w_t, dtype=np.float32)
    cout, k = w.shape
    if k % 32:
        raise LoweringError("split_pointwise_weights: k=%d must be a multiple of 32" % k)
    amax = np.abs(w).max(axis=1).astype(np.float64)
    e = np.zeros(cout, np.int64)
    nz = amax > 0
    e[nz] = 14 - np.frexp(amax[nz])[1]
    e = np.clip(e, -100, 100)
    ws = np.ldexp(w.astype(np.float64), e[:, None]).astype(np.float32)
    hi = ws.astype(np.float16)
    lo = (ws - hi.astype(np.float32)).astype(np.float16)
    assert np.isfinite(hi.astype(np.float32)).all()
    img = np.empty((cout, k // 32, 64), np.uint16)
    img[:, :, :32] = hi.view(np.uint16).reshape(cout, k // 32, 32)
    img[:, :, 32:] = lo.view(np.uint16).reshape(cout, k // 32, 32)
    descale = np.ldexp(np.ones(cout, np.float64), -(e + a_log2)).astype(np.float32)
    return img, descale


def stem4_conv_image(w_hwio: np.ndarray, in_log2: int, reverse_channels: bool = False) -> Tuple[np.ndarray, np.ndarray]:
    w = np.asarray(w_hwio, dtype=np.float32).reshape(3, 3, 3, 32)
    if reverse_channels:
        w = w[:, :, ::-1, :]
    w = w.reshape(3, 9, 32)
    full = np.zeros((32, 64), np.float32)
    for dy in range(3):
        full[:, 8 * dy:8 * dy + 8] = w[dy, :8, :].T
        full[:, 32 + 8 * dy] = w[dy, 8, :]
    img, ds = split_pointwise_weights(full, in_log2)
    return np.ascontiguousarray(img.transpose(1, 0, 2)), ds


def stem4_u8_shifts(w_hwio: np.ndarray, shift: np.ndarray, mean_bgr) -> np.ndarray:
    w = np.asarray(w_hwio, dtype=np.float64).reshape(3, 3, 3, 32)
    m = np.asarray(mean_bgr, dtype=np.float64).reshape(1, 1, 3, 1)
    out = np.zeros((4, 32), np.float64)
    for case in range(4):
        rows = 2 if case & 2 else 3
        cols = 2 if case & 1 else 3
        out[case] = np.asarray(shift, np.float64) - (w[:rows, :cols] * m).sum(axis=(0, 1, 2))
    return out.astype(np.float32)


def unsplit_pointwise_weights(img: np.ndarray, descale: np.ndarray, a_log2: int) -> np.ndarray:
    cout, kt, _ = img.shape
    hi = img[:, :, :32].copy().view(np.float16).astype(np.float64).reshape(cout, kt * 32)
    lo = img[:, :, 32:].copy().view(np.float16).astype(np.float64).reshape(cout, kt * 32)
    return (hi + lo) * (descale.astype(np.float64) * 2.0 ** a_log2)[:, None]


@dataclass
class Layer:
# ... 564 lines not shown
            raise LoweringError("%s: cannot fuse, input %s has %d consumers" % (node.name, acts[0][0].name, nconsumers))
        cout = L.out_shape[2]

        def vec(v):
            v = np.asarray(v, dtype=np.float32).reshape(-1)
            if v.size == 1:
                v = np.full(cout, v[0], np.float32)
            if v.size != cout:
                raise LoweringError("%s: operand of %d elements against %d channels" % (node.name, v.size, cout))
            return v

        if L.res >= 0 and op not in ("Relu", "Relu6", "Minimum", "Maximum"):
            raise LoweringError("%s: affine op after a fused residual sum" % node.name)
        if op in ("Mul",) and not L.sealed and L.act == ACT_NONE and L.kind in (OP_CONV_C3, OP_DWCONV3X3, OP_PWCONV_F32, OP_DENSE, OP_CONV_BF16, OP_STEM7X7_BF16, OP_CONV_F32):
            v = vec(consts[0])
            L.scale = v if L.scale is None else L.scale * v
            if L.shift is not None:
                L.shift = L.shift * v
        elif op in ("Add", "AddV2", "BiasAdd") and not L.sealed and L.act == ACT_NONE and L.kind in (OP_CONV_C3, OP_DWCONV3X3, OP_PWCONV_F32, OP_DENSE, OP_CONV_BF16, OP_STEM7X7_BF16, OP_CONV_F32):
            v = vec(consts[0])
            L.shift = v if L.shift is None else L.shift + v
        elif op == "Sub" and not L.sealed and L.act == ACT_NONE and ins[0][0] is acts[0][0]:
            v = vec(consts[0])
            L.shift = -v if L.shift is None else L.shift - v
        elif op in ("FusedBatchNorm", "FusedBatchNormV3") and not L.sealed and L.act == ACT_NONE:
            if node.attr_b("is_training", True):
                raise LoweringError("%s: training-mode FusedBatchNorm in a frozen graph" % node.name)
            gamma, beta, mean, var = [vec(c) for c in consts[:4]]
            k = gamma / np.sqrt(var + np.float32(node.attr_f("epsilon", 1e-3)))
            L.scale = k if L.scale is None else L.scale * k
            L.shift = (beta - mean * k) if L.shift is None else (L.shift * k + beta - mean * k)
        elif op == "Relu" and not L.sealed and L.act == ACT_NONE:
            L.act = ACT_RELU
        elif op == "Relu6" and not L.sealed and L.act == ACT_NONE:
            L.act = ACT_RELU6
        elif op == "Minimum" and not L.sealed and L.act == ACT_RELU and float(np.asarray(consts[0]).reshape(-1)[0]) == 6.0:
            L.act = ACT_RELU6
        elif op == "Maximum" and L.act in (ACT_RELU, ACT_RELU6) and float(np.asarray(consts[0]).reshape(-1)[0]) == 0.0:
            pass
        elif op == "Sigmoid" and not L.sealed and L.act == ACT_NONE and L.kind == OP_DENSE:
            L.act = ACT_SIGMOID
        else:
            raise LoweringError("%s: cannot fuse op %s into layer %s (act=%d sealed=%s)" %
                                (node.name, op, L.name, L.act, L.sealed))
        L.version += 1
        self.where[node.name] = idx
        return idx

    def is_final(self, name: str) -> bool:
        li = self.where[name]
        return li >= 0 and self.ver.get(name, 0) == self.layers[li].version


def assign_buffers(layers: List[Layer], pinned) -> List[int]:
    last_use = list(range(len(layers)))
    for i, L in enumerate(layers):
        for s in (L.src, L.res):
            if s >= 0:
                last_use[s] = i
    for i, L in enumerate(layers):
        span = 1 if L.flags & OPF_PAIR_NEXT else 3 if L.flags & OPF_HEADS else 0
        for j in range(i, min(i + span, len(layers) - 1) + 1 if span else i):
            for s in (layers[j].src, layers[j].res, j):
                if s >= 0:
                    last_use[s] = max(last_use[s], i + span)
    buffers: List[int] = []
    free: List[int] = []
    for i, L in enumerate(layers):
        need = L.out_bytes
        pick = None
        if i not in pinned and free:
            fits = [b for b in free if buffers[b] >= need]
            pick = min(fits, key=lambda b: buffers[b]) if fits else max(free, key=lambda b: buffers[b])
            free.remove(pick)
            buffers[pick] = max(buffers[pick], need)
        if pick is None:
            buffers.append(need)
            pick = len(buffers) - 1
        L.out_buf = pick
        for j in range(i + 1):
            if last_use[j] == i and j not in pinned and layers[j].out_buf not in free:
                free.append(layers[j].out_buf)
    for i, L in enumerate(layers):
        if L.flags & OPF_DWPW_NEXT and L.src >= 0 and i + 1 < len(layers) and layers[i + 1].out_buf == layers[L.src].out_buf:
            a, b = layers[L.src].out_buf, L.out_buf
            buffers[a] = buffers[b] = max(buffers[a], buffers[b])
    return buffers


def consumers_of(layers: List[Layer]) -> Dict[int, List[Tuple[int, str]]]:
    consumers: Dict[int, List[Tuple[int, str]]] = {}
    for i, L in enumerate(layers):
        for how in ("src", "res"):
            s = getattr(L, how)
            if s >= 0:
                consumers.setdefault(s, []).append((i, how))
    return consumers


def sole_reader(consumers: Dict[int, List[Tuple[int, str]]], i: int, keep: Sequence[int]) -> int:
    cons = consumers.get(i, [])
    return cons[0][0] if i not in keep and len(cons) == 1 and cons[0][1] == "src" else -1


def rebuild(layers: List[Layer], drop, put: Dict[int, Layer]) -> Tuple[List[Layer], Dict[int, int]]:
    new_layers: List[Layer] = []
    remap: Dict[int, int] = {}
    for i, L in enumerate(layers):
        if i in drop:
            remap[i] = -1
        else:
            remap[i] = len(new_layers)
            new_layers.append(put.get(i, L))
    for L in new_layers:
        for how in ("src", "res"):
            s = getattr(L, how)
            if s >= 0:
                if remap[s] < 0:
                    raise LoweringError("%s still reads %s (as %s), which a fusion pass removed" % (L.name, layers[s].name, how))
                setattr(L, how, remap[s])
    return new_layers, remap


def dwpw_fusable(dw: Layer, pw: Layer) -> bool:
    return (dw.kind == OP_DWCONV3X3 and pw.kind == OP_PWCONV_F32 and dw.act == ACT_RELU6 and pw.act == ACT_RELU6 and
            dw.in_shape[2] in (32, 64) and pw.out_shape[2] in (64, 128) and dw.stride in (1, 2))


def fuse_dwpw(layers: List[Layer], keep: Sequence[int]) -> Tuple[List[Layer], Dict[int, int]]:
    consumers = consumers_of(layers)
    put: Dict[int, Layer] = {}
    drop = set()
    for i, dw in enumerate(layers):
        j = sole_reader(consumers, i, keep)
        if dw.kind == OP_DWCONV3X3 and j >= 0 and dwpw_fusable(dw, layers[j]):
            pw = layers[j]
            put[j] = Layer(OP_DWPW_F32, pw.name, dw.src, dw.in_shape, pw.out_shape, w=dw.w, scale=dw.scale, shift=dw.shift,
                           act=pw.act, kh=3, kw=3, stride=dw.stride, pad_t=dw.pad_t, pad_l=dw.pad_l, sealed=True,
                           w2=pw.w, shift2=pw.shift)
            drop.add(i)
    return rebuild(layers, drop, put)


def fuse_stem_pool(layers: List[Layer], keep: Sequence[int]) -> Tuple[List[Layer], Dict[int, int]]:
    consumers = consumers_of(layers)
    for i, L in enumerate(layers):
        p = sole_reader(consumers, i, keep)
        if not (L.kind == OP_STEM7X7_BF16 and L.act == ACT_RELU and p >= 0):
            continue
        P = layers[p]
        oh, ow = L.out_shape[0], L.out_shape[1]
        if not (P.kind == OP_MAXPOOL_BF16 and P.pad_t in (0, 1) and P.pad_l in (0, 1) and
                2 * (P.out_shape[0] - 1) - P.pad_t < oh and 2 * (P.out_shape[1] - 1) - P.pad_l < ow):
            continue
        S = Layer(OP_STEM7X7_POOL_BF16, P.name, -1, L.in_shape, P.out_shape, w=L.w, scale=L.scale, shift=L.shift, act=ACT_RELU,
                  kh=7, kw=7, stride=2, pad_t=3, pad_l=3, sealed=True, pad3=(P.pad_t, P.pad_l), tensors=list(P.tensors))
        return rebuild(layers, {i}, {p: S})
    return rebuild(layers, set(), {})


def fuse_proj(layers: List[Layer], keep: Sequence[int]) -> Tuple[List[Layer], Dict[int, int]]:
    consumers = consumers_of(layers)
    drop = set()
    for i, P in enumerate(layers):
        cons = consumers.get(i, [])
        if not (P.kind == OP_CONV_BF16 and P.kh == 1 and P.kw == 1 and P.pad_t == 0 and P.pad_l == 0 and P.act == ACT_NONE and P.res < 0 and
                P.proj is None and P.src >= 0 and i not in keep and len(cons) == 1 and cons[0][1] == "res" and 1 <= P.stride <= 3):
# ... 119 lines not shown
        b = sole_reader(consumers, i, keep)
        if not (L.kind == OP_CONV_C3 and b >= 0 and L.src == -1 and L.in_shape[2] == 3 and
                L.out_shape[2] == 32 and L.stride == 2 and L.kh == 3 and L.kw == 3 and L.act == ACT_RELU6):
            continue
        B = layers[b]
        if not (B.kind == OP_DWPW_F32 and B.stride == 1 and B.in_shape[2] == 32 and B.out_shape[2] == 64):
            continue
        S = Layer(OP_STEM_F16S, B.name, -1, L.in_shape, B.out_shape, w=B.w, scale=B.scale, shift=B.shift, act=B.act, kh=3, kw=3,
                  stride=2, pad_t=L.pad_t, pad_l=L.pad_l, sealed=True, w2=B.w2, shift2=B.shift2, a_log2=F16S_ACT_LOG2_RELU6,
                  w0=L.w, shift0=L.shift)
        return rebuild(layers, {i}, {b: S})
    return rebuild(layers, set(), {})


def fuse_stem2(layers: List[Layer], keep: Sequence[int]) -> Tuple[List[Layer], Dict[int, int]]:
    consumers = consumers_of(layers)
    for i0, L0 in enumerate(layers):
        if not (L0.kind == OP_CONV_C3 and L0.src == -1 and L0.in_shape[2] == 3 and L0.out_shape[2] == 32 and L0.stride == 2 and
                L0.kh == 3 and L0.kw == 3 and L0.act == ACT_RELU6):
            continue
        i1 = sole_reader(consumers, i0, keep)
        if i1 < 0 or not (layers[i1].kind == OP_DWCONV3X3 and layers[i1].stride == 1 and layers[i1].act == ACT_RELU6):
            continue
        i2 = sole_reader(consumers, i1, keep)
        if i2 < 0 or not (layers[i2].kind == OP_PWCONV_F32 and layers[i2].out_shape[2] == 64 and layers[i2].act == ACT_RELU6):
            continue
        i3 = sole_reader(consumers, i2, keep)
        if i3 < 0 or not (layers[i3].kind == OP_DWCONV3X3 and layers[i3].stride == 2 and layers[i3].in_shape[2] == 64 and
                          layers[i3].act in (ACT_NONE, ACT_RELU, ACT_RELU6)):
            continue
        L1, L2, L3 = layers[i1], layers[i2], layers[i3]
        S = Layer(OP_STEM2_F16S, L3.name, -1, L0.in_shape, L3.out_shape, w=L1.w, scale=L1.scale, shift=L1.shift, act=L3.act, kh=3, kw=3,
                  stride=2, pad_t=L0.pad_t, pad_l=L0.pad_l, sealed=True, w2=L2.w, shift2=L2.shift, a_log2=F16S_ACT_LOG2_RELU6,
                  w0=L0.w, shift0=L0.shift, w3=L3.w, scale3=L3.scale, shift3=L3.shift, pad3=(L3.pad_t, L3.pad_l))
        return rebuild(layers, {i0, i1, i2}, {i3: S})
    return rebuild(layers, set(), {})


BLOCK_F16S_AUTO = ((128, 128), (256, 256))


def block_f16s_fusable(dw: Layer, pw: Layer, which: str) -> bool:
    c, cout = dw.in_shape[2], pw.out_shape[2]
    if not (dw.kind == OP_DWCONV3X3 and pw.kind == OP_PWCONV_F32 and pw.a_log2 > 0 and dw.act == ACT_RELU6 and
            pw.act in (ACT_NONE, ACT_RELU, ACT_RELU6) and dw.stride in (1, 2) and c % 32 == 0 and cout % 64 == 0):
        return False
    return which == "all" or (dw.stride == 1 and (c, cout) in BLOCK_F16S_AUTO)


def fuse_block_f16s(layers: List[Layer], keep: Sequence[int], which: str) -> Tuple[List[Layer], Dict[int, int]]:
    consumers = consumers_of(layers)
    put: Dict[int, Layer] = {}
    drop = set()
    for i, dw in enumerate(layers):
        j = sole_reader(consumers, i, keep)
        if dw.kind == OP_DWCONV3X3 and j >= 0 and block_f16s_fusable(dw, layers[j], which):
            pw = layers[j]
            put[j] = Layer(OP_DWPW_F16S, pw.name, dw.src, dw.in_shape, pw.out_shape, w=dw.w, scale=dw.scale, shift=dw.shift,
                           act=pw.act, kh=3, kw=3, stride=dw.stride, pad_t=dw.pad_t, pad_l=dw.pad_l, sealed=True,
                           w2=pw.w, shift2=pw.shift, a_log2=pw.a_log2)
            drop.add(i)
    return rebuild(layers, drop, put)


def dwpw_pair_covered(dw: Layer, pw: Layer) -> bool:
    return dw.stride == 2 and dw.in_shape[2] == 128 and pw.out_shape[2] == 256


def mark_dwpw_pairs(layers: List[Layer], keep: Sequence[int]) -> int:
    consumers = consumers_of(layers)
    n = 0
    for i, dw in enumerate(layers):
        j = sole_reader(consumers, i, keep)
        if not (dw.kind == OP_DWCONV3X3 and dw.act == ACT_RELU6 and dw.out_split == 0 and dw.flags == 0 and j == i + 1):
            continue
        pw = layers[j]
        if (pw.kind == OP_PWCONV_F32 and 0 < pw.a_log2 <= 12 and not pw.in_split and pw.flags == 0 and pw.res < 0 and
                tuple(pw.in_shape) == tuple(dw.out_shape) and dwpw_pair_covered(dw, pw)):
            dw.flags |= OPF_DWPW_NEXT
            n += 1
    return n


def choose_pointwise_math(layers: List[Layer], pw_math: str) -> None:
    if pw_math not in ("auto", "f32", "f16split"):
        raise ValueError("pw_math must be 'auto', 'f32' or 'f16split', not %r" % (pw_math,))
    if pw_math == "f32":
        return
    for L in layers:
        if L.kind != OP_PWCONV_F32:
            continue
        bounded = L.src >= 0 and layers[L.src].act == ACT_RELU6 and layers[L.src].kind not in _BF16_OUT
        if bounded and L.in_shape[2] % 32 == 0 and L.out_shape[2] % 64 == 0:
            L.a_log2 = F16S_ACT_LOG2_RELU6
        elif pw_math == "f16split":
            raise LoweringError("%s: split-f16 pointwise needs a ReLU6-bounded input, k %% 32 == 0 and cout %% 64 == 0" % L.name)


PRESPLIT_MIN_K = 256


def presplit_activations(layers: List[Layer], keep: Sequence[int]) -> int:
    consumers = consumers_of(layers)
    n = 0
    for i, L in enumerate(layers):
        if not (L.kind == OP_PWCONV_F32 and L.a_log2 > 0 and L.src >= 0):
            continue
        P = layers[L.src]
        k, cout = L.in_shape[2], L.out_shape[2]
        if (P.kind == OP_DWCONV3X3 and P.act == ACT_RELU6 and L.src not in keep and consumers.get(L.src) == [(i, "src")] and
                k % 32 == 0 and k >= PRESPLIT_MIN_K and cout % 128 == 0 and 0 < L.a_log2 <= 12):
            P.out_split = L.a_log2
            L.in_split = True
            n += 1
    return n


def pwdw_fusable(pw: Layer, dw: Layer) -> bool:
    h, w, _ = dw.in_shape
    if not (pw.kind == OP_PWCONV_F32 and pw.a_log2 > 0 and pw.in_split and pw.out_shape[2] % 128 == 0 and
            dw.kind == OP_DWCONV3X3 and dw.act == ACT_RELU6 and 0 < dw.out_split <= 12 and h * w <= 288):
        return False
    if dw.stride == 1:
        return dw.pad_t == 1 and dw.pad_l == 1 and dw.out_shape == dw.in_shape
    return (dw.stride == 2 and (h, w) in ((12, 12), (14, 14)) and (dw.pad_t, dw.pad_l) == (0, 0) and dw.out_shape[:2] == (h // 2, w // 2) and
            pw.act == ACT_RELU6)


def fuse_pwgap(layers: List[Layer], keep: Sequence[int]) -> Tuple[List[Layer], Dict[int, int]]:
    consumers = consumers_of(layers)
    for i, L in enumerate(layers):
        j = sole_reader(consumers, i, keep)
        h, w, c = L.out_shape
        if not (L.kind == OP_PWCONV_F32 and L.a_log2 > 0 and L.in_split and c % 128 == 0 and j >= 0 and
                layers[j].kind == OP_GAP and 33 <= h * w <= 288):
            continue
        G = layers[j]
        F = Layer(OP_PWGAP_PS, G.name, L.src, L.in_shape, G.out_shape, w=L.w, shift=L.shift, act=L.act, sealed=True, a_log2=L.a_log2,
                  in_split=True, tensors=list(G.tensors))
        return rebuild(layers, {i}, {j: F})
    return rebuild(layers, set(), {})


def fuse_pwdw(layers: List[Layer], keep: Sequence[int]) -> Tuple[List[Layer], Dict[int, int]]:
    consumers = consumers_of(layers)
    put: Dict[int, Layer] = {}
    drop = set()
    for i, pw in enumerate(layers):
        j = sole_reader(consumers, i, keep)
        if j >= 0 and pwdw_fusable(pw, layers[j]):
            dw = layers[j]
            put[j] = Layer(OP_PWDW_PS, dw.name, pw.src, pw.in_shape, dw.out_shape, w=pw.w, shift=pw.shift, act=pw.act, sealed=True,
                           a_log2=pw.a_log2, in_split=True, w3=dw.w, scale3=dw.scale, shift3=dw.shift, out_split=dw.out_split, kh=3, kw=3,
                           stride=dw.stride, pad_t=dw.pad_t, pad_l=dw.pad_l, tensors=list(dw.tensors))
            drop.add(i)
    return rebuild(layers, drop, put)


def lower_graph(g: Graph, input_tensor: str, outputs: Dict[int, str], input_hw: Optional[Tuple[int, int]] = None,
                feeds: Optional[Dict[str, object]] = None, fuse: bool = True, dtype: str = "f32",
                pw_math: Optional[str] = None, fuse_stem_block: Optional[bool] = None, stem_fusion: Optional[str] = None,
                block_fusion: Optional[str] = None, presplit: Optional[str] = None, input_bound: Optional[float] = None,
                pwdw_fusion: Optional[str] = None, u8_mean_bgr: Optional[Sequence[float]] = None, launch_fusion: bool = True,
                s2_fusion: Optional[str] = None) -> Plan:
    if dtype not in ("f32", "bf16", "f32g"):
        raise ValueError("dtype must be 'f32', 'bf16' or 'f32g', not %r" % (dtype,))
    in_node, _ = g.get_tensor_by_name(input_tensor)
    shape = g.placeholder_shape(in_node.name)
    if input_hw is None:
        if shape is None or len(shape) != 4 or shape[1] <= 0 or shape[2] <= 0:
            raise ValueError("input tensor %s has no static HxW; pass input_hw" % input_tensor)
        input_hw = (int(shape[1]), int(shape[2]))
    feeds_n = {}
    for k, v in (feeds or {}).items():
        feeds_n[g.get_tensor_by_name(k)[0].name] = v
    low = _Lowerer(g, in_node.name, input_hw, feeds_n, dtype)
    if shape is not None and len(shape) == 4 and shape[3] > 0:
        low.in_c = int(shape[3])
    out_layers: Dict[int, Tuple[int, int]] = {}
    low.mark_live([g.get_tensor_by_name(t)[0] for t in outputs.values()])
    for slot, tname in outputs.items():
        node, _ = g.get_tensor_by_name(tname)
        li = low.lower_node(node)
        if li < 0:
            raise LoweringError("output %s is the graph input" % tname)
        out_layers[slot] = (li, int(np.prod(low.layers[li].out_shape)))
    layers = low.layers

    for L in layers:
        if L.kind in (OP_CONV_C3, OP_PWCONV_F32, OP_DENSE) and L.scale is not None:
            L.w = (L.w * L.scale.reshape((1,) * (L.w.ndim - 1) + (-1,))).astype(np.float32)
            L.scale = None
        if L.kind in (OP_CONV_C3, OP_PWCONV_F32, OP_DWCONV3X3, OP_DENSE) and L.shift is None:
            L.shift = np.zeros(L.out_shape[2], np.float32)
        if L.kind == OP_DWCONV3X3 and L.scale is None:
            L.scale = np.ones(L.out_shape[2], np.float32)
        if L.kind == OP_CONV_F32 and L.act not in (ACT_NONE, ACT_RELU, ACT_RELU6):
            raise LoweringError("%s: activation %d on a general convolution" % (L.name, L.act))
        if L.kind in (OP_CONV_BF16, OP_STEM7X7_BF16):
            cout = L.out_shape[2]
            L.scale = np.ones(cout, np.float32) if L.scale is None else L.scale.astype(np.float32)
            L.shift = np.zeros(cout, np.float32) if L.shift is None else L.shift.astype(np.float32)
            if L.act not in (ACT_NONE, ACT_RELU, ACT_RELU6):
                raise LoweringError("%s: activation %d on a bf16 convolution" % (L.name, L.act))
            from .resnet50 import pack_conv_weight, pack_stem_weight
            L.w = pack_stem_weight(L.w) if L.kind == OP_STEM7X7_BF16 else pack_conv_weight(L.w)

    for slot, tname in outputs.items():
        nm = g.get_tensor_by_name(tname)[0].name
        if not low.is_final(nm):
            raise LoweringError("output %s is an intermediate of fused layer %s; fetch the layer's final tensor"
                                % (tname, layers[low.where[nm]].name))
    tensor_layer = {name: li for name, li in low.where.items() if li >= 0 and low.is_final(name)}

    def keep() -> List[int]:
        return [li for li, _ in out_layers.values()]

    def apply(fuse_pass, *args) -> None:
        nonlocal layers, out_layers, tensor_layer
        layers, remap = fuse_pass(layers, keep(), *args)
        out_layers = {slot: (remap[li], e) for slot, (li, e) in out_layers.items()}
        tensor_layer = {name: remap[li] for name, li in tensor_layer.items() if remap[li] >= 0}

    pw_math = pw_math or "auto"
    if stem_fusion is None:
        stem_fusion = "none" if fuse_stem_block is False else "stem2"
    if stem_fusion not in ("none", "stem", "stem2"):
        raise ValueError("stem_fusion must be 'none', 'stem' or 'stem2', not %r" % (stem_fusion,))
    want_stem = fuse and dtype == "f32" and pw_math != "f32" and stem_fusion != "none"
    if want_stem and stem_fusion == "stem2":
        apply(fuse_stem2)
        if input_bound is not None:
            if not (input_bound > 0 and np.isfinite(input_bound)):
                raise ValueError("input_bound must be a positive finite number, not %r" % (input_bound,))
            in_log2 = int(np.floor(np.log2(32768.0 / float(input_bound))))
            in_log2 = max(-8, min(14, in_log2))
            if float(input_bound) * 2.0 ** in_log2 <= 32768.0:
                for L in layers:
                    if L.kind == OP_STEM2_F16S:
                        L.kind, L.in_log2 = OP_STEM3_F16S, in_log2
                        if u8_mean_bgr is not None:
                            if len(u8_mean_bgr) != 3 or not all(0.0 <= float(m) <= 255.0 for m in u8_mean_bgr):
                                raise ValueError("u8_mean_bgr must be three means in [0, 255], not %r" % (u8_mean_bgr,))
                            if float(input_bound) < 256.0:
                                raise ValueError("uint8 input needs input_bound >= 256 (pixels minus a mean), not %r" % (input_bound,))
                            L.u8_mean_bgr = tuple(float(m) for m in u8_mean_bgr)
    if fuse and dtype == "bf16":
        for fuse_pass in (fuse_stem_pool, fuse_proj):
            apply(fuse_pass)
        subsample_stage_tails(layers, keep())
    if fuse:
        apply(fuse_dwpw)

    if dtype == "f32":
        choose_pointwise_math(layers, pw_math)
        if want_stem:
            apply(fuse_stem)
        block_fusion = block_fusion or "auto"
        if block_fusion not in ("auto", "none", "all"):
            raise ValueError("block_fusion must be 'auto', 'none' or 'all', not %r" % (block_fusion,))
        if fuse and block_fusion != "none":
            apply(fuse_block_f16s, block_fusion)
        presplit = presplit or "auto"
        if presplit not in ("auto", "none"):
            raise ValueError("presplit must be 'auto' or 'none', not %r" % (presplit,))
        if presplit == "auto":
            presplit_activations(layers, keep())
            pwdw_fusion = pwdw_fusion or "auto"
            if pwdw_fusion not in ("auto", "none"):
                raise ValueError("pwdw_fusion must be 'auto' or 'none', not %r" % (pwdw_fusion,))
            if fuse and pwdw_fusion == "auto":
                apply(fuse_pwdw)
                apply(fuse_pwgap)
    if fuse and launch_fusion:
        if dtype == "bf16":
            mark_pairs(layers)
            compact_pair_outputs(layers, keep())
        if dtype == "f32":
            mark_heads(layers)
    s2_fusion = s2_fusion or "auto"
    if s2_fusion not in ("auto", "none"):
        raise ValueError("s2_fusion must be 'auto' or 'none', not %r" % (s2_fusion,))
    if fuse and launch_fusion and dtype == "f32" and s2_fusion == "auto":
        mark_dwpw_pairs(layers, keep())
    buffers = assign_buffers(layers, set(keep()))
    return Plan(layers, (input_hw[0], input_hw[1], low.in_c), buffers, out_layers, tensor_layer)
```

### hse_facerec_tf_amd/ops.py

```python
from __future__ import annotations

import ctypes
from typing import Optional, Tuple

import numpy as np

from . import _lib
from .lowering import ACT_NONE, ACT_RELU, ACT_RELU6, ACT_SIGMOID, tf_same_padding


def _device_guarded(fn):
    import functools

    @functools.wraps(fn)
    def wrapper(*args, **kw):
        devs = [a.device for a in list(args) + list(kw.values()) if hasattr(a, "is_cuda") and a.is_cuda]
        if not devs:
            return fn(*args, **kw)
        if any(d != devs[0] for d in devs):
            raise ValueError("%s: tensors live on different devices: %s" % (fn.__name__, sorted({str(d) for d in devs})))
        with _lib.on_device(devs[0]):
            return fn(*args, **kw)
    return wrapper

# ... 90 lines not shown
    if not (xs.is_cuda and xs.dtype == torch.float16 and xs.is_contiguous() and xs.dim() == 6 and tuple(xs.shape[-2:]) == (2, 32)):
        raise ValueError("xs must be a contiguous float16 CUDA tensor [n, h, w, k/32, 2, 32]")
    d_img, d_ds = prepared if prepared is not None else split_weights_device(w_t, xs.device, a_log2)
    n, h, w = int(xs.shape[0]), int(xs.shape[1]), int(xs.shape[2])
    k, cout = xs.shape[3] * 32, d_img.shape[0]
    y = torch.empty((n, cout), dtype=torch.float32, device=xs.device)
    _lib.check(_lib.lib().hsefr_pwconv1x1_presplit_gap(xs.data_ptr(), d_img.data_ptr(), d_ds.data_ptr(), shift.data_ptr(), y.data_ptr(),
                                                       n * h * w, k, cout, act, h * w, _lib.current_stream_ptr()), "hsefr_pwconv1x1_presplit_gap")
    return y


@_device_guarded
def pwconv1x1_presplit_dw(xs, w_t, shift, dw_w_hwc, dw_scale, dw_shift, act: int = ACT_RELU6, a_log2: int = 12, out_log2: int = 12, prepared=None,
                          dw_stride: int = 1):
    torch = _lib.require_gpu()
    _f32c(shift, "shift"), _f32c(dw_w_hwc, "dw_w"), _f32c(dw_scale, "dw_scale"), _f32c(dw_shift, "dw_shift")
    if not (xs.is_cuda and xs.dtype == torch.float16 and xs.is_contiguous() and xs.dim() == 6 and tuple(xs.shape[-2:]) == (2, 32)):
        raise ValueError("xs must be a contiguous float16 CUDA tensor [n, h, w, k/32, 2, 32]")
    d_img, d_ds = prepared if prepared is not None else split_weights_device(w_t, xs.device, a_log2)
    n, h, w = int(xs.shape[0]), int(xs.shape[1]), int(xs.shape[2])
    k, cout = xs.shape[3] * 32, d_img.shape[0]
    if tuple(dw_w_hwc.shape) != (3, 3, cout) or dw_scale.numel() != cout or dw_shift.numel() != cout:
        raise ValueError("depthwise operands must be [3,3,%d], [%d], [%d]" % (cout, cout, cout))
    amp = float(2 ** out_log2)
    consts = torch.cat([dw_w_hwc.reshape(9, cout), (dw_scale * amp).reshape(1, cout), (dw_shift * amp).reshape(1, cout)]).contiguous()
    ys = torch.empty((n, h // dw_stride, w // dw_stride, cout // 32, 2, 32), dtype=torch.float16, device=xs.device)
    _lib.check(_lib.lib().hsefr_pwconv1x1_presplit_dw(xs.data_ptr(), d_img.data_ptr(), d_ds.data_ptr(), shift.data_ptr(), consts.data_ptr(),
                                                      ys.data_ptr(), n * h * w, k, cout, act, w, h * w, dw_stride, out_log2,
                                                      _lib.current_stream_ptr()),
               "hsefr_pwconv1x1_presplit_dw")
    return ys


@_device_guarded
def pwconv1x1(x, w_t, shift, act: int = ACT_RELU6):
    torch = _lib.require_gpu()
    _f32c(x, "x"), _f32c(w_t, "w_t"), _f32c(shift, "shift")
    k = x.shape[-1]
    cout = w_t.shape[0]
    m = x.numel() // k
    y = torch.empty(tuple(x.shape[:-1]) + (cout,), dtype=torch.float32, device=x.device)
    _lib.check(_lib.lib().hsefr_pwconv1x1_bias_relu6(x.data_ptr(), w_t.data_ptr(), shift.data_ptr(), y.data_ptr(),
                                                     m, k, cout, act, _lib.current_stream_ptr()),
               "hsefr_pwconv1x1_bias_relu6")
    return y


def split_weights_device(w_t, device, a_log2: int = 12):
    torch = _lib.require_gpu()
    from . import lowering
    w_np = w_t.detach().cpu().numpy() if hasattr(w_t, "detach") else w_t
    img, descale = lowering.split_pointwise_weights(w_np, a_log2)
    return torch.from_numpy(img.view(np.int16)).to(device), torch.from_numpy(descale).to(device)


@_device_guarded
def pwconv1x1_f16split(x, w_t, shift, act: int = ACT_RELU6, a_log2: int = 12, prepared=None):
    torch = _lib.require_gpu()
    _f32c(x, "x"), _f32c(shift, "shift")
    d_img, d_ds = prepared if prepared is not None else split_weights_device(w_t, x.device, a_log2)
    k = x.shape[-1]
    cout = d_img.shape[0]
    m = x.numel() // k
    y = torch.empty(tuple(x.shape[:-1]) + (cout,), dtype=torch.float32, device=x.device)
    _lib.check(_lib.lib().hsefr_pwconv1x1_f16split(x.data_ptr(), d_img.data_ptr(), d_ds.data_ptr(), shift.data_ptr(),
                                                   y.data_ptr(), m, k, cout, a_log2, act, _lib.current_stream_ptr()),
               "hsefr_pwconv1x1_f16split")
    return y


@_device_guarded
def dwpw_f16split(x, w_hwc, dscale, dshift, wp_t, pshift, stride: int = 1, act: int = ACT_RELU6, a_log2: int = 12, prepared=None):
    torch = _lib.require_gpu()
    for t, nm in ((x, "x"), (w_hwc, "w"), (dscale, "dscale"), (dshift, "dshift"), (pshift, "pshift")):
        _f32c(t, nm)
    d_img, d_ds = prepared if prepared is not None else split_weights_device(wp_t, x.device, a_log2)
    n, h, w, c = x.shape
    cout = d_img.shape[0]
    oh, ow, pt, pl = _same(h, w, 3, stride)
    y = torch.empty((n, oh, ow, cout), dtype=torch.float32, device=x.device)
    _lib.check(_lib.lib().hsefr_dwpw_f16split(x.data_ptr(), w_hwc.data_ptr(), dscale.data_ptr(), dshift.data_ptr(), d_img.data_ptr(),
                                              d_ds.data_ptr(), pshift.data_ptr(), y.data_ptr(), n, h, w, c, stride, pt, pl, oh, ow,
                                              cout, a_log2, act, _lib.current_stream_ptr()), "hsefr_dwpw_f16split")
    return y


@_device_guarded
def stem_fused(x, conv_w, conv_shift, w_hwc, dscale, dshift, wp_t, pshift, act: int = ACT_RELU6, a_log2: int = 12, prepared=None):
    torch = _lib.require_gpu()
    if not hasattr(_lib.lib(), "hsefr_stem_fused"):
        raise NotImplementedError("round 1's fused stem is part of DEVELOPMENT builds of the library only (HSEFR_LIB=libhsefr_dev.so)")
    for t, nm in ((x, "x"), (conv_w, "conv_w"), (conv_shift, "conv_shift"), (w_hwc, "w"), (dscale, "dscale"), (dshift, "dshift"),
                  (pshift, "pshift")):
        _f32c(t, nm)
    d_img, d_ds = prepared if prepared is not None else split_weights_device(wp_t, x.device, a_log2)
    n, h, w, c = x.shape
    if c != 3 or tuple(conv_w.shape) != (3, 3, 3, 32) or tuple(w_hwc.shape) != (3, 3, 32) or d_img.shape[0] != 64:
        raise NotImplementedError("stem_fused covers 3 -> 32 -> 64 channels")
    oh, ow, pt, pl = _same(h, w, 3, 2)
    y = torch.empty((n, oh, ow, 64), dtype=torch.float32, device=x.device)
    _lib.check(_lib.lib().hsefr_stem_fused(x.data_ptr(), conv_w.data_ptr(), conv_shift.data_ptr(), w_hwc.data_ptr(), dscale.data_ptr(),
                                           dshift.data_ptr(), d_img.data_ptr(), d_ds.data_ptr(), pshift.data_ptr(), y.data_ptr(),
                                           n, h, w, pt, pl, oh, ow, a_log2, act, _lib.current_stream_ptr()), "hsefr_stem_fused")
    return y


@_device_guarded
def stem2_fused(x, conv_w, conv_shift, w1_hwc, d1scale, d1shift, wp_t, pshift, w2_hwc, d2scale, d2shift, act: int = ACT_RELU6,
                a_log2: int = 12, prepared=None):
    torch = _lib.require_gpu()
    for t, nm in ((x, "x"), (conv_w, "conv_w"), (conv_shift, "conv_shift"), (w1_hwc, "w1"), (d1scale, "d1scale"), (d1shift, "d1shift"),
                  (pshift, "pshift"), (w2_hwc, "w2"), (d2scale, "d2scale"), (d2shift, "d2shift")):
        _f32c(t, nm)
    d_img, d_ds = prepared if prepared is not None else split_weights_device(wp_t, x.device, a_log2)
    n, h, w, c = x.shape
    if c != 3 or tuple(conv_w.shape) != (3, 3, 3, 32) or tuple(w1_hwc.shape) != (3, 3, 32) or d_img.shape[0] != 64 or \
            tuple(w2_hwc.shape) != (3, 3, 64):
        raise NotImplementedError("stem2_fused covers 3 -> 32 -> 64 channels")
    h1, w1, pt, pl = _same(h, w, 3, 2)
    oh2, ow2, pt2, pl2 = _same(h1, w1, 3, 2)
    y = torch.empty((n, oh2, ow2, 64), dtype=torch.float32, device=x.device)
    _lib.check(_lib.lib().hsefr_stem2_fused(x.data_ptr(), conv_w.data_ptr(), conv_shift.data_ptr(), w1_hwc.data_ptr(), d1scale.data_ptr(),
                                            d1shift.data_ptr(), d_img.data_ptr(), d_ds.data_ptr(), pshift.data_ptr(), w2_hwc.data_ptr(),
                                            d2scale.data_ptr(), d2shift.data_ptr(), y.data_ptr(), n, h, w, pt, pl, h1, w1, pt2, pl2,
                                            oh2, ow2, a_log2, act, _lib.current_stream_ptr()), "hsefr_stem2_fused")
    return y


@_device_guarded
def stem3_fused(x, conv_w, conv_shift, w1_hwc, d1scale, d1shift, wp_t, pshift, w2_hwc, d2scale, d2shift, act: int = ACT_RELU6,
                a_log2: int = 12, in_log2: int = 7, prepared=None, overflow=None):
    torch = _lib.require_gpu()
    from . import lowering
    for t, nm in ((x, "x"), (conv_shift, "conv_shift"), (w1_hwc, "w1"), (d1scale, "d1scale"), (d1shift, "d1shift"),
                  (pshift, "pshift"), (w2_hwc, "w2"), (d2scale, "d2scale"), (d2shift, "d2shift")):
        _f32c(t, nm)
    d_img, d_ds = prepared if prepared is not None else split_weights_device(wp_t, x.device, a_log2)
    n, h, w, c = x.shape
    cw = conv_w.detach().cpu().numpy() if hasattr(conv_w, "detach") else np.asarray(conv_w)
    if c != 3 or tuple(cw.shape) != (3, 3, 3, 32) or tuple(w1_hwc.shape) != (3, 3, 32) or d_img.shape[0] != 64 or tuple(w2_hwc.shape) != (3, 3, 64):
        raise NotImplementedError("stem3_fused covers 3 -> 32 -> 64 channels")
    cw_t = np.zeros((32, 32), np.float32)
    cw_t[:, :27] = cw.reshape(27, 32).T
    cimg, cds = lowering.split_pointwise_weights(cw_t, in_log2)
    d_cimg = torch.from_numpy(cimg.view(np.int16)).to(x.device)
    d_cds = torch.from_numpy(cds).to(x.device)
    h1, w1, pt, pl = _same(h, w, 3, 2)
    oh2, ow2, pt2, pl2 = _same(h1, w1, 3, 2)
    y = torch.empty((n, oh2, ow2, 64), dtype=torch.float32, device=x.device)
    _lib.check(_lib.lib().hsefr_stem3_fused(x.data_ptr(), d_cimg.data_ptr(), d_cds.data_ptr(), conv_shift.data_ptr(), w1_hwc.data_ptr(),
                                            d1scale.data_ptr(), d1shift.data_ptr(), d_img.data_ptr(), d_ds.data_ptr(), pshift.data_ptr(),
                                            w2_hwc.data_ptr(), d2scale.data_ptr(), d2shift.data_ptr(), y.data_ptr(),
                                            None if overflow is None else overflow.data_ptr(), n, h, w, pt, pl, h1, w1, pt2, pl2,
                                            oh2, ow2, in_log2, a_log2, act, _lib.current_stream_ptr()), "hsefr_stem3_fused")
    return y


def stem5_stream(*args, **kw):
    return stem4_fused(*args, _entry="hsefr_stem5_stream", **kw)


@_device_guarded
def stem4_fused(x, conv_w, conv_shift, w1_hwc, d1scale, d1shift, wp_t, pshift, w2_hwc, d2scale, d2shift, act: int = ACT_RELU6,
                a_log2: int = 12, in_log2: int = 7, prepared=None, overflow=None, u8_mean_bgr=None, _entry: str = "hsefr_stem4_fused"):
    torch = _lib.require_gpu()
    from . import lowering
# ... 752 lines not shown
```

### include/hsefr.h

```cpp
#ifndef HSEFR_H
#define HSEFR_H

#include <stddef.h>
#include <stdint.h>

#ifdef __cplusplus
extern "C" {
#endif

#define HSEFR_VERSION 141

typedef enum hsefr_status {
    HSEFR_OK = 0,
    HSEFR_ERR_INVALID = -1,
    HSEFR_ERR_UNSUPPORTED = -2,
    HSEFR_ERR_HIP = -3,
    HSEFR_ERR_NOMEM = -4,
    HSEFR_ERR_SHAPE = -5
} hsefr_status;

typedef enum hsefr_act {
    HSEFR_ACT_NONE = 0,
    HSEFR_ACT_RELU = 1,
    HSEFR_ACT_RELU6 = 2,
    HSEFR_ACT_SIGMOID = 3
} hsefr_act;

typedef void* hsefr_stream_t;

int hsefr_version(void);
const char* hsefr_last_error_string(void);

#define HSEFR_PLAN_MAGIC 0x314c505246455348ull
#define HSEFR_NO_OFFSET 0xffffffffffffffffull
#define HSEFR_BUF_INPUT (-1)
#define HSEFR_BUF_NONE (-2)

typedef enum hsefr_op_kind {
    HSEFR_OP_CONV_C3 = 1,
    HSEFR_OP_DWCONV3X3 = 2,
    HSEFR_OP_PWCONV_F32 = 3,
    HSEFR_OP_GAP = 4,
    HSEFR_OP_DENSE = 5,
    HSEFR_OP_SOFTMAX = 6,
    HSEFR_OP_CONV_BF16 = 7,
    HSEFR_OP_MAXPOOL_BF16 = 8,
    HSEFR_OP_GAP_BF16 = 9,
    HSEFR_OP_STEM7X7_BF16 = 10,
    HSEFR_OP_DWPW_F32 = 11,
    HSEFR_OP_PWCONV_F16S = 12,
    HSEFR_OP_DWPW_F16S = 13,
    HSEFR_OP_STEM_F16S = 14,
    HSEFR_OP_CONV_F32 = 18,
    HSEFR_OP_MAXPOOL_F32 = 19,
    HSEFR_OP_STEM7X7_POOL_BF16 = 20,
    HSEFR_OP_PWCONV_PS_DW = 21,
    HSEFR_OP_PWCONV_PS_GAP = 22,
    HSEFR_OP_STEM3_F16S = 17,
    HSEFR_OP_PWCONV_PS = 16,
    HSEFR_OP_STEM2_F16S = 15
} hsefr_op_kind;

typedef enum hsefr_output_slot {
    HSEFR_OUT_FEATURES = 0,
    HSEFR_OUT_AGE = 1,
    HSEFR_OUT_GENDER = 2,
    HSEFR_N_OUTPUT_SLOTS = 3
} hsefr_output_slot;

typedef struct hsefr_plan_header {
    uint64_t magic;
    uint32_t version;
    uint32_t n_buffers;
    uint32_t n_ops;
    uint32_t in_h, in_w, in_c;
    int32_t out_buffer[HSEFR_N_OUTPUT_SLOTS];
    uint32_t out_elems[HSEFR_N_OUTPUT_SLOTS];
    uint64_t blob_bytes;
} hsefr_plan_header;

typedef struct hsefr_plan_buffer {
    uint64_t elems_per_image;
    uint32_t elem_bytes;
    uint32_t reserved;
} hsefr_plan_buffer;

typedef enum hsefr_op_flags {
    HSEFR_OPF_PAIR_NEXT = 1,
    HSEFR_OPF_HEADS = 2,
    HSEFR_OPF_OUT_SUB2 = 4,
    HSEFR_OPF_DWPW_NEXT = 8
} hsefr_op_flags;

enum {
    HSEFR_AUX_C2_SHIFT = 0, HSEFR_AUX_C2_BITS = 12,
    HSEFR_AUX_STRIDE2_SHIFT = 12, HSEFR_AUX_STRIDE2_BITS = 2,
    HSEFR_AUX_H2_SHIFT = 14, HSEFR_AUX_H2_BITS = 9,
    HSEFR_AUX_W2_SHIFT = 23, HSEFR_AUX_W2_BITS = 9,
    HSEFR_AUX_LOG2_BITS = 8,
    HSEFR_AUX_OUT_LOG2_SHIFT = 8,
    HSEFR_AUX_IN_LOG2_SHIFT = 8,
    HSEFR_AUX_IN_LOG2_BIAS = 64,
    HSEFR_AUX_U8_BIT = 16,
    HSEFR_AUX_POOL_PAD_L_SHIFT = 4
};

enum { HSEFR_STEM_KW_PAD_T2_BIT = 4, HSEFR_STEM_KW_PAD_L2_BIT = 5 };

enum {
    HSEFR_STEM_PACK_CONV = 0,
    HSEFR_STEM_PACK_CONV_SHIFT = 864,
    HSEFR_STEM_PACK_DW1 = 896,
    HSEFR_STEM_PACK_DW1_SCALE = 1184,
    HSEFR_STEM_PACK_DW1_SHIFT = 1216,
    HSEFR_STEM_PACK_DW2 = 1248,
    HSEFR_STEM_PACK_DW2_SCALE = 1824,
    HSEFR_STEM_PACK_DW2_SHIFT = 1888,
    HSEFR_STEM_PACK_STEM2_END = 1952,
    HSEFR_STEM_PACK_CONV_SPLIT = 1952,
    HSEFR_STEM_PACK_CONV_DESCALE = 2976,
    HSEFR_STEM_PACK_CONV4 = 3008,
    HSEFR_STEM_PACK_CONV4_U8 = 5056,
    HSEFR_STEM_PACK_U8_SHIFT = 7104,
    HSEFR_STEM_PACK_U8_DESCALE = 7232,
    HSEFR_STEM_PACK_STEM3_END = 7264
};

enum { HSEFR_STEM_SHIFT2_DESCALE = 0, HSEFR_STEM_SHIFT2_SHIFT = 64 };

typedef struct hsefr_plan_op {
    uint32_t kind;
    uint32_t act;
    int32_t in_buf, out_buf, res_buf;
    int32_t h, w, cin;
    int32_t oh, ow, cout;
    int32_t kh, kw, stride;
    int32_t pad_t, pad_l;
    int32_t aux;
    int32_t flags;
    uint64_t w_off;
    uint64_t scale_off;
    uint64_t shift_off;
    uint64_t w2_off;
    uint64_t shift2_off;
} hsefr_plan_op;

typedef struct hsefr_engine hsefr_engine;

int hsefr_engine_create(const void* plan, size_t plan_bytes, int max_batch, hsefr_engine** out);

int hsefr_plan_validate(const void* plan, size_t plan_bytes);

int hsefr_plan_describe(const void* plan, size_t plan_bytes, int n, char* out, size_t out_bytes);

int hsefr_engine_set_graph_batch(hsefr_engine* e, int max_n);
long long hsefr_engine_graph_launches(const hsefr_engine* e);

size_t hsefr_engine_workspace_bytes(const hsefr_engine* e);
int hsefr_engine_max_batch(const hsefr_engine* e);

int hsefr_engine_forward(hsefr_engine* e, const void* d_input, int n, void* d_features,
                         void* d_age_probs, void* d_gender, hsefr_stream_t stream);

int hsefr_engine_accepts_u8(const hsefr_engine* e);
int hsefr_engine_forward_u8(hsefr_engine* e, const void* d_input_u8, int n, void* d_features, void* d_age_probs, void* d_gender,
                            hsefr_stream_t stream);

void* hsefr_engine_buffer(hsefr_engine* e, int buffer);
int hsefr_engine_copy_buffer(hsefr_engine* e, int buffer, void* d_dst, size_t bytes, hsefr_stream_t stream);

int hsefr_engine_set_profiling(hsefr_engine* e, int depth);
long long hsefr_engine_profiled_calls(const hsefr_engine* e);
int hsefr_engine_op_times_ms(hsefr_engine* e, int slot, float* ms, int n_ops);

int hsefr_engine_input_overflow(hsefr_engine* e, int* host_flag, hsefr_stream_t stream);
int hsefr_engine_input_overflow_async(hsefr_engine* e, int* pinned_host_flag, hsefr_stream_t stream);
int hsefr_engine_destroy(hsefr_engine* e);


int hsefr_conv_c3_bias_act(const float* x, const float* wgt, const float* shift, float* y, int n, int h,
                           int w, int kh, int kw, int stride, int pad_t, int pad_l, int oh, int ow,
                           int cout, int act, hsefr_stream_t stream);

int hsefr_dwconv3x3_bn_relu6(const float* x, const float* wgt, const float* scale, const float* shift,
                             float* y, int n, int h, int w, int c, int stride, int pad_t, int pad_l,
                             int oh, int ow, int act, hsefr_stream_t stream);

int hsefr_dwconv3x3_bn_relu6_split(const float* x, const float* wgt, const float* scale, const float* shift, void* y_split,
                                   int n, int h, int w, int c, int stride, int pad_t, int pad_l, int oh, int ow, int act,
                                   int a_log2, hsefr_stream_t stream);

int hsefr_pwconv1x1_bias_relu6(const float* x, const float* wgt_t, const float* shift, float* y,
                               long long m, int k, int cout, int act, hsefr_stream_t stream);

int hsefr_pwconv1x1_f16split(const float* x, const void* w_split, const float* descale, const float* shift, float* y,
                             long long m, int k, int cout, int a_log2, int act, hsefr_stream_t stream);

int hsefr_pwconv1x1_presplit(const void* x_split, const void* w_split, const float* descale, const float* shift, float* y,
                             long long m, int k, int cout, int act, hsefr_stream_t stream);

int hsefr_pwconv1x1_presplit_gap(const void* x_split, const void* w_split, const float* descale, const float* shift, float* y,
                                 long long m, int k, int cout, int act, int map_hw, hsefr_stream_t stream);

int hsefr_pwconv1x1_presplit_dw(const void* x_split, const void* w_split, const float* descale, const float* shift, const float* dw_consts,
                                void* y_split, long long m, int k, int cout, int act, int map_w, int map_hw, int dw_stride, int out_log2,
                                hsefr_stream_t stream);

int hsefr_dwpw_f16split(const float* x, const float* wd, const float* dscale, const float* dshift, const void* w_split,
                        const float* descale, const float* pshift, float* y, int n, int h, int w, int c, int stride,
                        int pad_t, int pad_l, int oh, int ow, int cout, int a_log2, int act, hsefr_stream_t stream);

int hsefr_stem2_fused(const float* x, const float* conv_w, const float* conv_shift, const float* wd1, const float* d1scale,
                      const float* d1shift, const void* w_split, const float* descale, const float* pshift, const float* wd2,
                      const float* d2scale, const float* d2shift, float* y, int n, int h, int w, int cpad_t, int cpad_l,
                      int h1, int w1, int pad_t2, int pad_l2, int oh2, int ow2, int a_log2, int act, hsefr_stream_t stream);

int hsefr_stem3_fused(const float* x, const void* cw_split, const float* cdescale, const float* conv_shift, const float* wd1,
                      const float* d1scale, const float* d1shift, const void* w_split, const float* descale, const float* pshift,
                      const float* wd2, const float* d2scale, const float* d2shift, float* y, int* d_overflow, int n, int h, int w,
                      int cpad_t, int cpad_l, int h1, int w1, int pad_t2, int pad_l2, int oh2, int ow2, int in_log2, int a_log2,
                      int act, hsefr_stream_t stream);

int hsefr_stem4_fused(const void* x, int x_is_u8, const void* cw4, const float* cdescale, const float* conv_shift, const float* wd1,
                      const float* d1scale, const float* d1shift, const void* w_split, const float* descale, const float* pshift,
                      const float* wd2, const float* d2scale, const float* d2shift, float* y, int* d_overflow, int n, int h, int w,
                      int in_log2, int a_log2, int act, hsefr_stream_t stream);
int hsefr_stem5_stream(const void* x, int x_is_u8, const void* cw4, const float* cdescale, const float* conv_shift, const float* wd1,
                      const float* d1scale, const float* d1shift, const void* w_split, const float* descale, const float* pshift,
                      const float* wd2, const float* d2scale, const float* d2shift, float* y, int* d_overflow, int n, int h, int w,
                      int in_log2, int a_log2, int act, hsefr_stream_t stream);

int hsefr_dwpw_fused(const float* x, const float* wd, const float* dscale, const float* dshift, const float* wp_t,
                     const float* pshift, float* y, int n, int h, int w, int c, int stride, int pad_t, int pad_l, int oh,
                     int ow, int cout, hsefr_stream_t stream);

int hsefr_gap(const float* x, float* y, int n, int hw, int c, hsefr_stream_t stream);

int hsefr_dense(const float* x, const float* wgt, const float* bias, float* y, int n, int k, int cout,
                int act, hsefr_stream_t stream);

int hsefr_softmax(const float* x, float* y, int n, int c, hsefr_stream_t stream);

int hsefr_heads_fused(const float* x, const float* w1, const float* b1, const float* wa, const float* ba, const float* wg, const float* bg,
                      float* hidden, float* logits, float* age_probs, float* gender, int n, int k, int a, hsefr_stream_t stream);


int hsefr_conv_bf16(const void* x, const void* wgt_t, const float* scale, const float* shift, const void* res, void* y,
                    int n, int h, int w, int c, int oh, int ow, int cout, int kh, int kw, int stride, int pad_t,
                    int pad_l, int act, hsefr_stream_t stream);

int hsefr_conv1x1_proj_bf16(const void* x, const void* wgt_t, const float* scale, const float* shift, const void* x2, const void* wgt2_t,
                            const float* scale2, const float* shift2, void* y, int n, int oh, int ow, int c, int cout, int c2, int stride2,
                            int h2, int w2, int act, hsefr_stream_t stream);

int hsefr_conv1x1_sres_bf16(const void* x, const void* wgt_t, const float* scale, const float* shift, const void* res, void* y, int n, int oh,
                            int ow, int c, int cout, int res_stride, int h2, int w2, int act, hsefr_stream_t stream);

int hsefr_conv1x1_pair_bf16(const void* x, const void* w1_t, const float* scale1, const float* shift1, const void* res, const void* x2,
                            const void* wp_t, const float* scale_p, const float* shift_p, void* y1, const void* w2_t, const float* scale2,
                            const float* shift2, void* y2, long long pixels, int c, int cout1, int cout2, int c2, int act1, int act2,
                            hsefr_stream_t stream);

int hsefr_conv1x1_pair_sub2_bf16(const void* x, const void* w1_t, const float* scale1, const float* shift1, const void* res, const void* x2,
                                 const void* wp_t, const float* scale_p, const float* shift_p, void* y1, const void* w2_t, const float* scale2,
                                 const float* shift2, void* y2, int n, int h, int w, int c, int cout1, int cout2, int c2, int act1, int act2,
                                 hsefr_stream_t stream);

int hsefr_stem7x7_bf16(const float* x, const void* wgt_t, const float* scale, const float* shift, void* y, int n, int h,
                       int w, int oh, int ow, int act, hsefr_stream_t stream);

int hsefr_maxpool3x3s2_bf16(const void* x, void* y, int n, int h, int w, int c, int oh, int ow, int pad_t, int pad_l,
                            hsefr_stream_t stream);

int hsefr_gap_bf16(const void* x, float* y, int n, int hw, int c, hsefr_stream_t stream);


typedef enum hsefr_color_mode { HSEFR_COLOR_BGR_MEAN_F64 = 0, HSEFR_COLOR_RGB_UNIT = 1, HSEFR_COLOR_BGR_MEAN_F32 = 2,
                                HSEFR_COLOR_NONE_U8 = 3 } hsefr_color_mode;

int hsefr_preprocess_pil_u8(const unsigned char* d_in, unsigned char* d_tmp, float* d_out, int n, int H, int W, int oh, int ow,
                            const int* d_xmin, const int* d_xcnt, const int* d_xcoef, int xksize, const int* d_ymin,
                            const int* d_ycnt, const int* d_ycoef, int yksize, int color_mode, const double* mean3,
                            hsefr_stream_t stream);

int hsefr_preprocess_cv_u8(const unsigned char* d_in, float* d_out, int n, int H, int W, int oh, int ow, const int* d_x0,
                           const int* d_x1, const int* d_wx1, const int* d_y0, const int* d_y1, const int* d_wy1,
                           int color_mode, const double* mean3, hsefr_stream_t stream);

int hsefr_l2_normalize(const float* x, float* y, int n, int d, hsefr_stream_t stream);

int hsefr_nn1(const float* q, const float* g, int nq, int ng, int d, int* nn_index, float* nn_dist2,
              hsefr_stream_t stream);
int hsefr_knn(const float* q, const float* g, int nq, int ng, int d, int k, int* nn_index, float* nn_dist2, const int* g_label, int* pred,
              hsefr_stream_t stream);
// ... 82 lines not shown
```

Measured before the change: 246,100.

## Fuse pointwise conv with following depthwise-pointwise block in a streaming kernel

Adds a new streaming kernel that chains a 64->128 split-f16 pointwise conv, a 3x3 depthwise conv and a 128->128 pointwise conv in one launch. Rows flow through an LDS ring with wave specialization: loader/depthwise waves on one side, MFMA waves on the other. This keeps the 128-channel intermediate tensor out of global memory and removes a launch. The lowering marks eligible layer pairs by default, and the plan validator and the buffer-size logic are extended to match. In exchange it adds a large, specialized kernel with a heavy LDS footprint, 512 threads per block at one block per CU, which may limit occupancy.

```diff
diff --git a/hse_facerec_tf_amd/_lib.py b/hse_facerec_tf_amd/_lib.py
--- a/hse_facerec_tf_amd/_lib.py
+++ b/hse_facerec_tf_amd/_lib.py
@@ -45,6 +45,7 @@
     "hsefr_engine_input_overflow": (c_int, [c_void_p, POINTER(c_int), c_void_p]),
     "hsefr_engine_input_overflow_async": (c_int, [c_void_p, POINTER(c_int), c_void_p]),
     "hsefr_dwpw_f16split": (c_int, [_fp, _fp, _fp, _fp, c_void_p, _fp, _fp, _fp] + [c_int] * 12 + [c_void_p]),
+    "hsefr_pwblk_f16split": (c_int, [_fp, c_void_p, _fp, _fp, _fp, _fp, _fp, c_void_p, _fp, _fp, _fp, _fp] + [c_int] * 10 + [c_void_p]),
     "hsefr_pwconv1x1_f16split": (c_int, [_fp, c_void_p, _fp, _fp, _fp, c_longlong, c_int, c_int, c_int, c_int, c_void_p]),
     "hsefr_dwpw_fused": (c_int, [_fp] * 7 + [c_int] * 10 + [c_void_p]),
     "hsefr_gap": (c_int, [_fp, _fp, c_int, c_int, c_int, c_void_p]),
diff --git a/hse_facerec_tf_amd/csrc/common.h b/hse_facerec_tf_amd/csrc/common.h
--- a/hse_facerec_tf_amd/csrc/common.h
+++ b/hse_facerec_tf_amd/csrc/common.h
@@ -273,6 +273,10 @@
 bool dwpw_f16s_supported(int c, int cout, int stride);
 bool dwpw_s2_covered(int c, int cout, int stride);
 bool dwpw_s2_off();
+bool pwblk_covered(int cin, int cmid, int cout, int w);
+int launch_pwblk_f16s(const float* x, const void* w2split, const float* descale2, const float* shift2, const float* wd, const float* dscale,
+                      const float* dshift, const void* w3split, const float* descale3, const float* shift3, float* y, int n, int h, int w,
+                      int a_log2, int a_log2_blk, int act, int segs, hipStream_t s);
 int launch_stem_fused(const float* x, const float* cw, const float* cshift, const float* wd, const float* dscale,
                       const float* dshift, const void* wsplit, const float* descale, const float* pshift, float* y, int n,
                       int h, int w, int cpad_t, int cpad_l, int oh, int ow, int a_log2, int act, hipStream_t s);
diff --git a/hse_facerec_tf_amd/csrc/engine.hip b/hse_facerec_tf_amd/csrc/engine.hip
--- a/hse_facerec_tf_amd/csrc/engine.hip
+++ b/hse_facerec_tf_amd/csrc/engine.hip
@@ -291,7 +291,7 @@
     }
     for (uint32_t i = 0; i < h.n_ops; ++i) {
         const hsefr_plan_op& o = ops[i];
-        HSEFR_REQUIRE((o.flags & ~(HSEFR_OPF_PAIR_NEXT | HSEFR_OPF_HEADS | HSEFR_OPF_OUT_SUB2 | HSEFR_OPF_DWPW_NEXT)) == 0, HSEFR_ERR_INVALID,
+        HSEFR_REQUIRE((o.flags & ~(HSEFR_OPF_PAIR_NEXT | HSEFR_OPF_HEADS | HSEFR_OPF_OUT_SUB2 | HSEFR_OPF_DWPW_NEXT | HSEFR_OPF_PWBLK_NEXT)) == 0, HSEFR_ERR_INVALID,
                       "plan op %u: unknown flags 0x%x", i, o.flags);
         HSEFR_REQUIRE(!(o.flags & HSEFR_OPF_OUT_SUB2) || (o.flags & HSEFR_OPF_PAIR_NEXT), HSEFR_ERR_INVALID, "plan op %u: OUT_SUB2 without PAIR_NEXT", i);
         if (o.flags & HSEFR_OPF_PAIR_NEXT) {
@@ -337,6 +337,31 @@
             for (int sl = 0; sl < HSEFR_N_OUTPUT_SLOTS; ++sl)
                 HSEFR_REQUIRE(h.out_buffer[sl] != o.out_buf && (b.out_buf != o.in_buf || h.out_buffer[sl] != o.in_buf), HSEFR_ERR_INVALID,
                               "plan op %u: DWPW_NEXT: the depthwise tensor (or the buffer it exchanges roles with) is output slot %d", i, sl);
+        }
+        if (o.flags & HSEFR_OPF_PWBLK_NEXT) {
+            HSEFR_REQUIRE(o.flags == HSEFR_OPF_PWBLK_NEXT && i + 1 < h.n_ops, HSEFR_ERR_INVALID, "plan op %u: PWBLK_NEXT on the last op or beside another flag", i);
+            const hsefr_plan_op& b = ops[i + 1];
+            HSEFR_REQUIRE(o.kind == HSEFR_OP_PWCONV_F16S && o.act == HSEFR_ACT_RELU6 && o.res_buf == HSEFR_BUF_NONE && o.aux > 0 && o.aux <= 12 &&
+                              b.kind == HSEFR_OP_DWPW_F16S && b.stride == 1 && b.pad_t == 1 && b.pad_l == 1 && b.in_buf == o.out_buf && b.flags == 0 &&
+                              b.h == o.h && b.w == o.w && b.oh == b.h && b.ow == b.w && b.cin == o.cout,
+                          HSEFR_ERR_INVALID, "plan op %u: PWBLK_NEXT needs a split-f16 pointwise op with ReLU6 and no residual (a_log2 in [1, 12]), and behind "
+                          "it a stride-1 split-f16 depthwise-pointwise block without flags that reads it at the same pixels", i);
+            HSEFR_REQUIRE(pwblk_covered(o.cin, o.cout, b.cout, o.w), HSEFR_ERR_INVALID,
+                          "plan op %u: PWBLK_NEXT %d -> %d -> %d channels on rows of %d pixels not covered (64 -> 128 -> 128, at most 48)", i, o.cin, o.cout,
+                          b.cout, o.w);
+            HSEFR_REQUIRE(b.out_buf != o.out_buf, HSEFR_ERR_INVALID, "plan op %u: PWBLK_NEXT: the second output (buffer %d) aliases the pointwise tensor", i,
+                          b.out_buf);
+            HSEFR_REQUIRE(b.out_buf != o.in_buf || (o.in_buf >= 0 && (uint64_t)bufs[o.in_buf].elems_per_image * bufs[o.in_buf].elem_bytes ==
+                                                                        (uint64_t)bufs[o.out_buf].elems_per_image * bufs[o.out_buf].elem_bytes),
+                          HSEFR_ERR_INVALID, "plan op %u: PWBLK_NEXT: buffers %d and %d exchange roles and must have one size", i, o.in_buf, o.out_buf);
+            for (uint32_t k = i + 2; k < h.n_ops; ++k) {
+                HSEFR_REQUIRE(ops[k].in_buf != o.out_buf && ops[k].res_buf != o.out_buf, HSEFR_ERR_INVALID,
+                              "plan op %u: PWBLK_NEXT: op %u also reads the pointwise tensor (buffer %d)", i, k, o.out_buf);
+                if (ops[k].out_buf == o.out_buf) break;
+            }
+            for (int sl = 0; sl < HSEFR_N_OUTPUT_SLOTS; ++sl)
+                HSEFR_REQUIRE(h.out_buffer[sl] != o.out_buf && (b.out_buf != o.in_buf || h.out_buffer[sl] != o.in_buf), HSEFR_ERR_INVALID,
+                              "plan op %u: PWBLK_NEXT: the pointwise tensor (or the buffer it exchanges roles with) is output slot %d", i, sl);
         }
         if (o.flags & HSEFR_OPF_HEADS) {
             HSEFR_REQUIRE(i + 3 < h.n_ops, HSEFR_ERR_INVALID, "plan op %u: HEADS needs three ops behind it", i);
@@ -685,6 +710,14 @@
         covered = 1;
         return launch_dwpw_f16s((const float*)in, (const float*)p.w, p.scale, p.shift, pb.w, pb.scale, pb.shift, (float*)tab[b.out_buf], n, o.h, o.w,
                                 o.cin, o.stride, o.pad_t, o.pad_l, o.oh, o.ow, b.cout, b.aux, b.act, s);
+    }
+    if ((o.flags & HSEFR_OPF_PWBLK_NEXT) && !every_tensor && needed[i + 1]) {
+        const hsefr_plan_op& b = e->ops[i + 1];
+        const Operands pb = operands(e, b);
+        if (b.out_buf == o.in_buf) std::swap(tab[o.in_buf], tab[o.out_buf]);
+        covered = 1;
+        return launch_pwblk_f16s((const float*)in, p.w, p.scale, p.shift, (const float*)pb.w, pb.scale, pb.shift, pb.w2, pb.shift2, pb.shift2 + b.cout,
+                                 (float*)tab[b.out_buf], n, o.h, o.w, o.aux, b.aux, b.act, 0, s);
     }
     const void* res = o.res_buf >= 0 ? tab[o.res_buf] : nullptr;
     switch (o.kind) {
@@ -1097,6 +1130,20 @@
                             a_log2, act, (hipStream_t)stream);
 }
 
+int hsefr_pwblk_f16split(const float* x, const void* w2_split, const float* descale2, const float* shift2, const float* wd, const float* dscale,
+                         const float* dshift, const void* w3_split, const float* descale3, const float* shift3, float* mid, float* y, int n, int h,
+                         int w, int cin, int cmid, int cout, int a_log2, int a_log2_blk, int act, int segs, hsefr_stream_t stream) {
+    HSEFR_REQUIRE(n == 0 || (x && w2_split && descale2 && shift2 && wd && dscale && dshift && w3_split && descale3 && shift3 && y), HSEFR_ERR_INVALID,
+                  "pwblk_f16split: null pointer");
+    if (pwblk_covered(cin, cmid, cout, w))
+        return launch_pwblk_f16s(x, w2_split, descale2, shift2, wd, dscale, dshift, w3_split, descale3, shift3, y, n, h, w, a_log2, a_log2_blk, act, segs,
+                                 (hipStream_t)stream);
+    HSEFR_REQUIRE(n == 0 || mid, HSEFR_ERR_INVALID, "pwblk_f16split: %d -> %d -> %d channels on rows of %d pixels take two launches and need `mid`", cin, cmid,
+                  cout, w);
+    if (int rc = launch_pwconv_f16s(x, w2_split, descale2, shift2, mid, (long long)n * h * w, cin, cmid, a_log2, HSEFR_ACT_RELU6, (hipStream_t)stream)) return rc;
+    return launch_dwpw_f16s(mid, wd, dscale, dshift, w3_split, descale3, shift3, y, n, h, w, cmid, 1, 1, 1, h, w, cout, a_log2_blk, act, (hipStream_t)stream);
+}
+
 int hsefr_dwpw_fused(const float* x, const float* wd, const float* dscale, const float* dshift, const float* wp_t,
                      const float* pshift, float* y, int n, int h, int w, int c, int stride, int pad_t, int pad_l, int oh,
                      int ow, int cout, hsefr_stream_t stream) {
diff --git a/hse_facerec_tf_amd/csrc/fuzz_plan.cc b/hse_facerec_tf_amd/csrc/fuzz_plan.cc
--- a/hse_facerec_tf_amd/csrc/fuzz_plan.cc
+++ b/hse_facerec_tf_amd/csrc/fuzz_plan.cc
@@ -53,7 +53,7 @@
 int main(int argc, char** argv) {
     if (argc < 3) { fprintf(stderr, "usage: fuzz_plan <mutants per seed> <plan file>...\n"); return 2; }
     const long long per_seed = atoll(argv[1]);
-    static const int32_t edge32[] = {0, 1, -1, -2, -3, 2, 3, 7, 8, 63, 64, 65, 127, 128, 255, 256, 511, 512, 4095, 4096, 65535, 65536, 0x7fffffff,
+    static const int32_t edge32[] = {0, 1, -1, -2, -3, 2, 3, 7, 8, 16, 24, 48, 49, 63, 64, 65, 127, 128, 255, 256, 511, 512, 4095, 4096, 65535, 65536, 0x7fffffff,
                                      (int32_t)0x80000000, (int32_t)0xffff0000, 1 << 20, 1 << 24, 1 << 30};
     static const uint64_t edge64[] = {0ull, 1ull, 15ull, 16ull, 17ull, 0xffffffffull, 0x100000000ull, 0x7fffffffffffffffull, 0x8000000000000000ull,
                                       0xffffffffffffffffull, 0xfffffffffffffff0ull};
diff --git a/hse_facerec_tf_amd/csrc/pwblk_stream.hip b/hse_facerec_tf_amd/csrc/pwblk_stream.hip
--- /dev/null
+++ b/hse_facerec_tf_amd/csrc/pwblk_stream.hip
@@ -0,0 +1,391 @@
+#include "common.h"
+
+#ifndef PB_ABLATE
+#define PB_ABLATE 0
+#endif
+namespace hsefr {
+
+namespace {
+
+typedef float f32x4 __attribute__((ext_vector_type(4)));
+typedef float f32x16 __attribute__((ext_vector_type(16)));
+typedef _Float16 f16x4 __attribute__((ext_vector_type(4)));
+typedef _Float16 f16x8 __attribute__((ext_vector_type(8)));
+
+constexpr int PB_CIN = 64, PB_C = 128, PB_COUT = 128;
+constexpr int PB_WMAX = 48;
+constexpr unsigned PB_GRID = 256;
+constexpr int PB_ROWB = 128;
+constexpr int PB_CELLB = PB_C * 4;
+constexpr int PB_RING = (PB_WMAX + 2) * PB_CELLB;
+constexpr int PB_KT = PB_WMAX * PB_ROWB;
+constexpr int PB_A2 = (PB_CIN / 32) * PB_KT, PB_A3 = (PB_C / 32) * PB_KT;
+constexpr int PB_A2_OFF = 2 * PB_RING, PB_A3_OFF = PB_A2_OFF + 2 * PB_A2, PB_S_OFF = PB_A3_OFF + 2 * PB_A3;
+constexpr int PB_ITEMS = 64;
+constexpr int PB_E_OFF = PB_S_OFF + 4 * 8192, PB_T_OFF = PB_E_OFF + 2 * PB_C * 4, PB_LDS = PB_T_OFF + PB_ITEMS * 16;
+static_assert(PB_LDS <= 160 * 1024, "LDS budget");
+
+struct PwBlkParams {
+    const float* x;
+    const float* w2;
+    const float* ds2;
+    const float* sh2;
+    const f32x4* wd;
+    const f32x4* dscale;
+    const f32x4* dshift;
+    const float* w3;
+    const float* ds3;
+    const float* sh3;
+    float* y;
+    int nimg, H, W, S;
+    unsigned total;
+    float a_scale2, a_scale3;
+    int reverse;
+    int act;
+    hsefr_udiv kS;
+};
+
+__device__ __forceinline__ int swzb(int row, int chunk) { return row * PB_ROWB + 16 * (chunk ^ ((row >> 1) & 7) ^ ((row & 1) << 2)); }
+__device__ __forceinline__ float relu6(float v) { return fminf(fmaxf(v, 0.f), 6.f); }
+__device__ __forceinline__ int ringb(int cell, int chunk) { return cell * PB_CELLB + 16 * (chunk ^ (cell & 7)); }
+
+constexpr int NB = 2;
+
+__global__ __launch_bounds__(512, 1) void pwblk_stream_f16s_kernel(PwBlkParams p) {
+    __shared__ __attribute__((aligned(1024))) unsigned char smem[PB_LDS];
+    const int tid = threadIdx.x;
+    const int lane = tid & 63;
+    const int wave = __builtin_amdgcn_readfirstlane(tid >> 6);
+    const int H = p.H, W = p.W;
+    const unsigned OOB = 0xFFFFFFF0u;
+    for (int i = tid; i < 2 * PB_RING / 16; i += 512) ((f32x4*)smem)[i] = f32x4{0.f, 0.f, 0.f, 0.f};
+    {
+        float* el = (float*)(smem + PB_E_OFF);
+        if (tid < PB_C) { el[tid] = p.ds2[tid]; el[PB_C + tid] = p.sh2[tid]; }
+    }
+    const unsigned nitem = (p.total - blockIdx.x + gridDim.x - 1) / gridDim.x;
+    int* itab = (int*)(smem + PB_T_OFF);
+    if (tid < (int)nitem) {
+        const unsigned lt = xcd_remap_dir(blockIdx.x + (unsigned)tid * gridDim.x, p.total, p.reverse);
+        const bool one = p.S == 1;
+        const unsigned n = one ? lt : hsefr_udiv_do(lt, p.kS), seg = lt - n * (unsigned)p.S;
+        const int r0 = one ? 0 : (int)hsefr_udiv_do(seg * (unsigned)H, p.kS);
+        itab[4 * tid] = (int)n;
+        itab[4 * tid + 1] = r0;
+        itab[4 * tid + 2] = (one ? H : (int)hsefr_udiv_do((seg + 1u) * (unsigned)H, p.kS)) - r0 + 2;
+    }
+    __syncthreads();
+    struct Cur { unsigned i; int s, R, n, r0; };
+    auto open = [&](Cur& c) {
+        const int* e = itab + 4 * (c.i < nitem ? c.i : nitem - 1);
+        c.n = __builtin_amdgcn_readfirstlane(e[0]);
+        c.r0 = __builtin_amdgcn_readfirstlane(e[1]);
+        c.R = __builtin_amdgcn_readfirstlane(e[2]);
+        c.s = 0;
+    };
+    auto next = [&](Cur& c) {
+        if (++c.s == c.R) { ++c.i; open(c); }
+    };
+    int nflat = 0;
+    for (unsigned i = 0; i < nitem; ++i) nflat += __builtin_amdgcn_readfirstlane(itab[4 * i + 2]);
+    const int nsteps = nflat + 3;
+    __syncthreads();
+
+    if (wave < 4) {
+        const __amdgpu_buffer_rsrc_t rx = make_rsrc(p.x, (long long)p.nimg * H * W * PB_CIN * 4);
+        unsigned xv[3];
+        int a2o[3];
+#pragma unroll
+        for (int j = 0; j < 3; ++j) {
+            const int i = tid + 256 * j;
+            xv[j] = i < W * 16 ? (unsigned)i * 16u : OOB;
+            const int cq = i & 15, skq = cq & 7;
+            a2o[j] = (cq >> 3) * PB_KT + swzb(i >> 4, skq >> 1) + 8 * (skq & 1);
+        }
+        f32x4 xr[3];
+        Cur cl;
+        cl.i = 0;
+        open(cl);
+        auto gload = [&]() {
+            const int q = cl.r0 - 1 + cl.s;
+            const bool ok = q >= 0 && q < H;
+            const unsigned so = __builtin_amdgcn_readfirstlane(ok ? (unsigned)((cl.n * H + q) * W) * (unsigned)(PB_CIN * 4) : 0u);
+#pragma unroll
+            for (int j = 0; j < 3; ++j) xr[j] = bload16(rx, ok ? xv[j] : OOB, so);
+            next(cl);
+        };
+        auto split = [&](unsigned char* At) {
+#pragma unroll
+            for (int j = 0; j < 3; ++j) {
+                const f32x4 v = xr[j] * p.a_scale2;
+                const f16x4 hi = __builtin_convertvector(v, f16x4);
+                const f16x4 lo = __builtin_convertvector(v - __builtin_convertvector(hi, f32x4), f16x4);
+                *(f16x4*)(At + a2o[j]) = hi;
+                *(f16x4*)(At + (a2o[j] ^ 64)) = lo;
+            }
+        };
+        const int quad = tid & 31, pg = tid >> 5;
+        f32x4 wk[9];
+#pragma unroll
+        for (int i = 0; i < 9; ++i) wk[i] = p.wd[i * (PB_C / 4) + quad];
+        const f32x4 dsc = p.dscale[quad], dsh = p.dshift[quad];
+        int ro[3];
+#pragma unroll
+        for (int t = 0; t < 3; ++t) ro[t] = ringb(pg + t, quad);
+        const int a3e = (quad >> 3) * PB_KT + swzb(pg, (quad & 7) >> 1) + 8 * (quad & 1);
+        f32x4 top[6], mid[6];
+#pragma unroll
+        for (int j = 0; j < 6; ++j) top[j] = mid[j] = f32x4{0.f, 0.f, 0.f, 0.f};
+        auto depthwise = [&](const unsigned char* rs, unsigned char* At) {
+#pragma unroll
+            for (int j = 0; j < 6; ++j) {
+                const f32x4 h0 = *(const f32x4*)(rs + ro[0] + j * 8 * PB_CELLB), h1 = *(const f32x4*)(rs + ro[1] + j * 8 * PB_CELLB),
+                            h2 = *(const f32x4*)(rs + ro[2] + j * 8 * PB_CELLB);
+                auto row_sum = [&](int b) {
+                    f32x4 t = h0 * wk[b];
+                    t = __builtin_elementwise_fma(h1, wk[b + 1], t);
+                    return __builtin_elementwise_fma(h2, wk[b + 2], t);
+                };
+                const f32x4 sa = row_sum(0), sb = row_sum(3), sc = row_sum(6);
+                const f32x4 sacc = mid[j] + sc;
+                mid[j] = top[j] + sb;
+                top[j] = sa;
+                const f32x4 o = __builtin_elementwise_fma(sacc, dsc, dsh);
+                f32x4 v;
+#pragma unroll
+                for (int e = 0; e < 4; ++e) v[e] = relu6(o[e]);
+                v = v * p.a_scale3;
+                const f16x4 hi = __builtin_convertvector(v, f16x4);
+                const f16x4 lo = __builtin_convertvector(v - __builtin_convertvector(hi, f32x4), f16x4);
+                const int ao = (a3e ^ (64 * (j & 1))) + j * 8 * PB_ROWB;
+                *(f16x4*)(At + ao) = hi;
+                *(f16x4*)(At + (ao ^ 64)) = lo;
+            }
+        };
+        gload();
+#pragma nounroll
+        for (int g = 0; g < nsteps; ++g) {
+            if (!(PB_ABLATE & 4)) {
+                if (g < nflat) split(smem + PB_A2_OFF + (g & 1) * PB_A2);
+                gload();
+            }
+            if (!(PB_ABLATE & 2) && g >= 2 && g < nflat + 2) depthwise(smem + (g & 1) * PB_RING, smem + PB_A3_OFF + (g & 1) * PB_A3);
+            __syncthreads();
+        }
+    } else {
+        const int cw = wave - 4;
+        const int li = lane & 31, lh = lane >> 5;
+        const int erow = lane >> 3, ech = lane & 7;
+        const __amdgpu_buffer_rsrc_t ry = make_rsrc(p.y, (long long)p.nimg * H * W * PB_COUT * 4);
+        f16x8 w2h[4], w2l[4], w3h[8], w3l[8];
+        {
+            const unsigned char* r2 = (const unsigned char*)p.w2 + (size_t)(32 * cw + li) * (PB_CIN * 4);
+            const unsigned char* r3 = (const unsigned char*)p.w3 + (size_t)(32 * cw + li) * (PB_C * 4);
+#pragma unroll
+            for (int s = 0; s < 4; ++s) {
+                w2h[s] = *(const f16x8*)(r2 + (s >> 1) * 128 + (2 * (s & 1) + lh) * 16);
+                w2l[s] = *(const f16x8*)(r2 + (s >> 1) * 128 + 64 + (2 * (s & 1) + lh) * 16);
+            }
+#pragma unroll
+            for (int s = 0; s < 8; ++s) {
+                w3h[s] = *(const f16x8*)(r3 + (s >> 1) * 128 + (2 * (s & 1) + lh) * 16);
+                w3l[s] = *(const f16x8*)(r3 + (s >> 1) * 128 + 64 + (2 * (s & 1) + lh) * 16);
+            }
+        }
+        f32x4 ds3 = *(const f32x4*)(p.ds3 + 32 * cw + 4 * ech), sh3 = *(const f32x4*)(p.sh3 + 32 * cw + 4 * ech);
+#pragma unroll
+        for (int s = 0; s < 4; ++s) asm volatile("" : "+v"(w2h[s]), "+v"(w2l[s]));
+#pragma unroll
+        for (int s = 0; s < 8; ++s) asm volatile("" : "+v"(w3h[s]), "+v"(w3l[s]));
+        asm volatile("" : "+v"(ds3), "+v"(sh3));
+        const float* el = (const float*)(smem + PB_E_OFF);
+        unsigned char* scr = smem + PB_S_OFF + cw * 8192;
+        Cur c1, c3;
+        c1.i = 0;
+        open(c1);
+        c3 = c1;
+        f32x16 acc2[NB], acc3[NB];
+        f16x8 fh[2][NB], fl[2][NB];
+        auto zero = [&](f32x16* acc) {
+#pragma unroll
+            for (int b = 0; b < NB; ++b)
+#pragma unroll
+                for (int r = 0; r < 16; ++r) acc[b][r] = 0.f;
+        };
+        auto fragments = [&](const unsigned char* St, int s, int buf) {
+            const unsigned char* row = St + (s >> 1) * PB_KT;
+#pragma unroll
+            for (int b = 0; b < NB; ++b) {
+                fh[buf][b] = *(const f16x8*)(row + swzb(b * 32 + li, 2 * (s & 1) + lh));
+                fl[buf][b] = *(const f16x8*)(row + swzb(b * 32 + li, 4 + 2 * (s & 1) + lh));
+            }
+        };
+        auto mfmas = [&](f32x16* acc, const f16x8& wh, const f16x8& wl, int buf) {
+#pragma unroll
+            for (int b = 0; b < NB; ++b) {
+                acc[b] = __builtin_amdgcn_mfma_f32_32x32x16_f16(wh, fl[buf][b], acc[b], 0, 0, 0);
+                acc[b] = __builtin_amdgcn_mfma_f32_32x32x16_f16(wl, fh[buf][b], acc[b], 0, 0, 0);
+                acc[b] = __builtin_amdgcn_mfma_f32_32x32x16_f16(wh, fh[buf][b], acc[b], 0, 0, 0);
+            }
+        };
+        auto product3 = [&](const unsigned char* St) {
+            zero(acc3);
+            fragments(St, 0, 0);
+#pragma unroll
+            for (int s = 0; s < 8; ++s) {
+                if (s + 1 < 8) fragments(St, s + 1, (s + 1) & 1);
+                mfmas(acc3, w3h[s], w3l[s], s & 1);
+            }
+        };
+        unsigned sv[NB][4];
+        f32x4 rv[4];
+        auto out_park = [&](int b) {
+#pragma unroll
+            for (int j = 0; j < 4; ++j) {
+                f32x4 v;
+#pragma unroll
+                for (int e = 0; e < 4; ++e) v[e] = acc3[b][4 * j + e];
+                *(f32x4*)(scr + b * 4096 + li * 128 + 16 * ((2 * j + lh) ^ (li & 7))) = v;
+            }
+        };
+        auto out_fetch = [&](int b) {
+#pragma unroll
+            for (int i = 0; i < 4; ++i) {
+                const int rr = erow + 8 * i;
+                rv[i] = *(const f32x4*)(scr + b * 4096 + rr * 128 + 16 * (ech ^ (rr & 7)));
+            }
+        };
+        auto out_store = [&](int b) {
+            f32x4 o[4];
+#pragma unroll
+            for (int i = 0; i < 4; ++i) o[i] = __builtin_elementwise_fma(rv[i], ds3, sh3);
+            if (p.act == HSEFR_ACT_RELU6) {
+#pragma unroll
+                for (int i = 0; i < 4; ++i)
+#pragma unroll
+                    for (int e = 0; e < 4; ++e) o[i][e] = apply_act<HSEFR_ACT_RELU6>(o[i][e]);
+            } else if (p.act == HSEFR_ACT_RELU) {
+#pragma unroll
+                for (int i = 0; i < 4; ++i)
+#pragma unroll
+                    for (int e = 0; e < 4; ++e) o[i][e] = apply_act<HSEFR_ACT_RELU>(o[i][e]);
+            }
+#pragma unroll
+            for (int i = 0; i < 4; ++i)
+                if (!(PB_ABLATE & 8)) bstore16_welded(o[i], ry, sv[b][i], 0u);
+        };
+#pragma nounroll
+        for (int g = 0; g < nsteps; ++g) {
+            const int par = (g + 1) & 1;
+            const bool emit = !(PB_ABLATE & 1) && g >= 3 && g < nflat + 3 && c3.s >= 2;
+            const bool feed = !(PB_ABLATE & 1) && g >= 1 && g < nflat + 1;
+            const int q = c1.r0 - 1 + c1.s;
+            const bool inside = feed && q >= 0 && q < H;
+            unsigned char* slot = smem + par * PB_RING;
+            const unsigned char* A2s = smem + PB_A2_OFF + par * PB_A2;
+            if (emit) {
+                const int r = c3.r0 + c3.s - 2;
+#pragma unroll
+                for (int b = 0; b < NB; ++b)
+#pragma unroll
+                    for (int i = 0; i < 4; ++i) {
+                        const int px = b * 32 + erow + 8 * i;
+                        sv[b][i] = px < W ? ((unsigned)((c3.n * H + r) * W + px) * (unsigned)PB_COUT + (unsigned)(32 * cw + 4 * ech)) * 4u : OOB;
+                    }
+                product3(smem + PB_A3_OFF + par * PB_A3);
+                out_park(0);
+                out_park(1);
+            }
+            if (inside) {
+                zero(acc2);
+                fragments(A2s, 0, 0);
+                fragments(A2s, 1, 1);
+                mfmas(acc2, w2h[0], w2l[0], 0);
+            }
+            if (emit) out_fetch(0);
+            if (inside) {
+                fragments(A2s, 2, 0);
+                mfmas(acc2, w2h[1], w2l[1], 1);
+            }
+            if (emit) { out_store(0); out_fetch(1); }
+            if (inside) {
+                fragments(A2s, 3, 1);
+                mfmas(acc2, w2h[2], w2l[2], 0);
+            }
+            if (emit) out_store(1);
+            if (inside) mfmas(acc2, w2h[3], w2l[3], 1);
+            if (inside) {
+                f32x4 ds[4], sh[4];
+#pragma unroll
+                for (int j = 0; j < 4; ++j) {
+                    ds[j] = *(const f32x4*)(el + 32 * cw + 8 * j + 4 * lh);
+                    sh[j] = *(const f32x4*)(el + PB_C + 32 * cw + 8 * j + 4 * lh);
+                }
+#pragma unroll
+                for (int b = 0; b < NB; ++b)
+#pragma unroll
+                    for (int j = 0; j < 4; ++j) {
+                        f32x4 v;
+#pragma unroll
+                        for (int e = 0; e < 4; ++e) v[e] = relu6(fmaf(acc2[b][4 * j + e], ds[j][e], sh[j][e]));
+                        if (b * 32 + li < W) *(f32x4*)(slot + ringb(b * 32 + li + 1, 8 * cw + 2 * j + lh)) = v;
+                    }
+            } else if (feed) {
+#pragma unroll
+                for (int b = 0; b < NB; ++b)
+#pragma unroll
+                    for (int j = 0; j < 4; ++j)
+                        if (b * 32 + li < W) *(f32x4*)(slot + ringb(b * 32 + li + 1, 8 * cw + 2 * j + lh)) = f32x4{0.f, 0.f, 0.f, 0.f};
+            }
+            if (!(PB_ABLATE & 1) && g >= 3 && g < nflat + 3) next(c3);
+            if (feed) next(c1);
+            __syncthreads();
+        }
+    }
+}
+
+}
+
+bool pwblk_covered(int cin, int cmid, int cout, int w) { return cin == PB_CIN && cmid == PB_C && cout == PB_COUT && w >= 1 && w <= PB_WMAX; }
+
+int launch_pwblk_f16s(const float* x, const void* w2split, const float* descale2, const float* shift2, const float* wd, const float* dscale,
+                      const float* dshift, const void* w3split, const float* descale3, const float* shift3, float* y, int n, int h, int w,
+                      int a_log2, int a_log2_blk, int act, int segs, hipStream_t s) {
+    HSEFR_REQUIRE(n >= 0 && h > 0 && w > 0 && w <= PB_WMAX, HSEFR_ERR_UNSUPPORTED, "pwblk_f16split: map %d x %d not covered (rows of at most %d pixels)",
+                  h, w, PB_WMAX);
+    HSEFR_REQUIRE(a_log2 > 0 && a_log2 <= 12 && a_log2_blk > 0 && a_log2_blk <= 12, HSEFR_ERR_INVALID, "pwblk_f16split: a_log2=%d / %d (1..12)", a_log2,
+                  a_log2_blk);
+    HSEFR_REQUIRE(segs >= 0, HSEFR_ERR_INVALID, "pwblk_f16split: segs=%d", segs);
+    if (n == 0) return HSEFR_OK;
+    HSEFR_REQUIRE((long long)n * h * w * PB_COUT * 4 < (1ll << 32) - 16, HSEFR_ERR_UNSUPPORTED, "pwblk_f16split: tensors beyond 4 GB");
+    PwBlkParams p;
+    p.x = x; p.w2 = (const float*)w2split; p.ds2 = descale2; p.sh2 = shift2;
+    p.wd = (const f32x4*)wd; p.dscale = (const f32x4*)dscale; p.dshift = (const f32x4*)dshift;
+    p.w3 = (const float*)w3split; p.ds3 = descale3; p.sh3 = shift3; p.y = y;
+    p.nimg = n; p.H = h; p.W = w;
+    int S = segs;
+    if (S == 0) {
+        const int fill = (int)((PB_GRID + (unsigned)n - 1) / (unsigned)n), most = h / 4 > 1 ? h / 4 : 1;
+        S = fill < most ? fill : most;
+    }
+    p.S = S < h ? S : h;
+    if (p.S > PB_ITEMS) p.S = PB_ITEMS;
+    p.kS = hsefr_udiv_make(p.S >= 2 ? (unsigned)p.S : 2u);
+    p.a_scale2 = ldexpf(1.f, a_log2);
+    p.a_scale3 = ldexpf(1.f, a_log2_blk);
+    p.reverse = sweep_reverse();
+    HSEFR_REQUIRE(act == HSEFR_ACT_RELU6 || act == HSEFR_ACT_RELU || act == HSEFR_ACT_NONE, HSEFR_ERR_UNSUPPORTED, "pwblk_f16split: act %d", act);
+    p.act = act;
+    const int per = (int)(PB_GRID * PB_ITEMS) / p.S;
+    for (int n0 = 0; n0 < n; n0 += per) {
+        p.nimg = n - n0 < per ? n - n0 : per;
+        p.x = x + (size_t)n0 * h * w * PB_CIN;
+        p.y = y + (size_t)n0 * h * w * PB_COUT;
+        p.total = (unsigned)p.nimg * (unsigned)p.S;
+        const unsigned g = p.total < PB_GRID ? p.total : PB_GRID;
+        HSEFR_LAUNCH(pwblk_stream_f16s_kernel, dim3(g), dim3(512), 0, s, p);
+    }
+    return launch_status("pwblk_f16split");
+}
+
+}
diff --git a/hse_facerec_tf_amd/lowering.py b/hse_facerec_tf_amd/lowering.py
--- a/hse_facerec_tf_amd/lowering.py
+++ b/hse_facerec_tf_amd/lowering.py
@@ -30,7 +30,7 @@
 _HEADER = struct.Struct("<QIIIIII3i3IQ")
 _BUFFER = struct.Struct("<QII")
 _OP = struct.Struct("<II3i3i3i3i2iii5Q")
-OPF_PAIR_NEXT, OPF_HEADS, OPF_OUT_SUB2, OPF_DWPW_NEXT = 1, 2, 4, 8
+OPF_PAIR_NEXT, OPF_HEADS, OPF_OUT_SUB2, OPF_DWPW_NEXT, OPF_PWBLK_NEXT = 1, 2, 4, 8, 16
 AUX_C2_SHIFT, AUX_C2_BITS, AUX_STRIDE2_SHIFT, AUX_STRIDE2_BITS = 0, 12, 12, 2
 AUX_H2_SHIFT, AUX_H2_BITS, AUX_W2_SHIFT, AUX_W2_BITS = 14, 9, 23, 9
 AUX_LOG2_BITS, AUX_OUT_LOG2_SHIFT, AUX_IN_LOG2_SHIFT, AUX_IN_LOG2_BIAS, AUX_U8_BIT = 8, 8, 8, 64, 16
@@ -46,7 +46,7 @@
 PRODUCT_KERNEL_FAMILIES = frozenset({
     "stem5_stream_kernel", "stem4_fused_kernel", "stem3_fused_kernel", "stem2_fused_kernel", "conv3x3_c3_kernel", "conv3x3_c3_mfma_kernel",
     "dwconv3x3_kernel", "pwconv_f32_dma_kernel", "pwconv_f32_kernel", "pwconv_f16s_kernel", "pwconv_ps_kernel", "dwpw_fused_kernel",
-    "dwpw_f16s_kernel", "dwpw2_f16s_kernel", "dwpw3_f16s_kernel", "dwpws2_f16s_kernel", "gap_kernel", "dense_kernel", "softmax_kernel", "heads_kernel",
+    "dwpw_f16s_kernel", "dwpw2_f16s_kernel", "dwpw3_f16s_kernel", "dwpws2_f16s_kernel", "pwblk_stream_f16s_kernel", "gap_kernel", "dense_kernel", "softmax_kernel", "heads_kernel",
     "stem7s_stream_kernel", "stem7x7_pool_bf16_kernel", "stem7x7_bf16_kernel", "maxpool3x3s2_bf16_kernel", "conv_bf16_kernel", "conv1x1_bf16_kernel",
     "conv1x1_w4_bf16_kernel", "conv1x1_pair_bf16_kernel", "conv3x3_w2_bf16_kernel", "conv_dma_bf16_kernel", "gap_bf16_kernel",
     "conv_f32_mfma_kernel", "conv2d_f32_kernel", "maxpool_f32_kernel"})
@@ -777,7 +777,7 @@
             if last_use[j] == i and j not in pinned and layers[j].out_buf not in free:
                 free.append(layers[j].out_buf)
     for i, L in enumerate(layers):
-        if L.flags & OPF_DWPW_NEXT and L.src >= 0 and i + 1 < len(layers) and layers[i + 1].out_buf == layers[L.src].out_buf:
+        if L.flags & (OPF_DWPW_NEXT | OPF_PWBLK_NEXT) and L.src >= 0 and i + 1 < len(layers) and layers[i + 1].out_buf == layers[L.src].out_buf:
             a, b = layers[L.src].out_buf, L.out_buf
             buffers[a] = buffers[b] = max(buffers[a], buffers[b])
     return buffers
@@ -1063,6 +1063,29 @@
     return n
 
 
+PW_BLOCK_MAX_W = 48
+
+
+def pw_block_covered(pw: Layer, blk: Layer) -> bool:
+    return pw.in_shape[2] == 64 and pw.out_shape[2] == 128 and blk.out_shape[2] == 128 and pw.out_shape[1] <= PW_BLOCK_MAX_W
+
+
+def mark_pw_blocks(layers: List[Layer], keep: Sequence[int]) -> int:
+    consumers = consumers_of(layers)
+    n = 0
+    for i, pw in enumerate(layers):
+        j = sole_reader(consumers, i, keep)
+        if not (pw.kind == OP_PWCONV_F32 and 0 < pw.a_log2 <= 12 and not pw.in_split and pw.flags == 0 and pw.res < 0 and pw.act == ACT_RELU6 and
+                j == i + 1):
+            continue
+        blk = layers[j]
+        if (blk.kind == OP_DWPW_F16S and blk.stride == 1 and (blk.pad_t, blk.pad_l) == (1, 1) and blk.flags == 0 and
+                tuple(blk.in_shape) == tuple(pw.out_shape) and tuple(blk.out_shape[:2]) == tuple(blk.in_shape[:2]) and pw_block_covered(pw, blk)):
+            pw.flags |= OPF_PWBLK_NEXT
+            n += 1
+    return n
+
+
 def choose_pointwise_math(layers: List[Layer], pw_math: str) -> None:
     if pw_math not in ("auto", "f32", "f16split"):
         raise ValueError("pw_math must be 'auto', 'f32' or 'f16split', not %r" % (pw_math,))
@@ -1143,7 +1166,7 @@
                 pw_math: Optional[str] = None, fuse_stem_block: Optional[bool] = None, stem_fusion: Optional[str] = None,
                 block_fusion: Optional[str] = None, presplit: Optional[str] = None, input_bound: Optional[float] = None,
                 pwdw_fusion: Optional[str] = None, u8_mean_bgr: Optional[Sequence[float]] = None, launch_fusion: bool = True,
-                s2_fusion: Optional[str] = None) -> Plan:
+                s2_fusion: Optional[str] = None, pw_block_fusion: Optional[str] = None) -> Plan:
     if dtype not in ("f32", "bf16", "f32g"):
         raise ValueError("dtype must be 'f32', 'bf16' or 'f32g', not %r" % (dtype,))
     in_node, _ = g.get_tensor_by_name(input_tensor)
@@ -1264,5 +1287,10 @@
         raise ValueError("s2_fusion must be 'auto' or 'none', not %r" % (s2_fusion,))
     if fuse and launch_fusion and dtype == "f32" and s2_fusion == "auto":
         mark_dwpw_pairs(layers, keep())
+    pw_block_fusion = pw_block_fusion or "auto"
+    if pw_block_fusion not in ("auto", "none"):
+        raise ValueError("pw_block_fusion must be 'auto' or 'none', not %r" % (pw_block_fusion,))
+    if fuse and launch_fusion and dtype == "f32" and pw_block_fusion == "auto":
+        mark_pw_blocks(layers, keep())
     buffers = assign_buffers(layers, set(keep()))
     return Plan(layers, (input_hw[0], input_hw[1], low.in_c), buffers, out_layers, tensor_layer)
diff --git a/hse_facerec_tf_amd/ops.py b/hse_facerec_tf_amd/ops.py
--- a/hse_facerec_tf_amd/ops.py
+++ b/hse_facerec_tf_amd/ops.py
@@ -196,6 +196,28 @@
     _lib.check(_lib.lib().hsefr_dwpw_f16split(x.data_ptr(), w_hwc.data_ptr(), dscale.data_ptr(), dshift.data_ptr(), d_img.data_ptr(),
                                               d_ds.data_ptr(), pshift.data_ptr(), y.data_ptr(), n, h, w, c, stride, pt, pl, oh, ow,
                                               cout, a_log2, act, _lib.current_stream_ptr()), "hsefr_dwpw_f16split")
+    return y
+
+
+@_device_guarded
+def pwblk_f16split(x, w2_t, shift2, w_hwc, dscale, dshift, w3_t, shift3, act: int = ACT_RELU6, a_log2: int = 12, a_log2_blk: int = 12, segs: int = 0,
+                   prepared2=None, prepared3=None):
+    torch = _lib.require_gpu()
+    for t, nm in ((x, "x"), (shift2, "shift2"), (w_hwc, "w"), (dscale, "dscale"), (dshift, "dshift"), (shift3, "shift3")):
+        _f32c(t, nm)
+    img2, ds2 = prepared2 if prepared2 is not None else split_weights_device(w2_t, x.device, a_log2)
+    img3, ds3 = prepared3 if prepared3 is not None else split_weights_device(w3_t, x.device, a_log2_blk)
+    n, h, w, cin = x.shape
+    cmid, cout = img2.shape[0], img3.shape[0]
+    if tuple(w_hwc.shape) != (3, 3, cmid) or dscale.numel() != cmid or dshift.numel() != cmid or shift2.numel() != cmid or shift3.numel() != cout:
+        raise ValueError("depthwise operands must be [3,3,%d], [%d], [%d]; shifts [%d], [%d]" % (cmid, cmid, cmid, cmid, cout))
+    y = torch.empty((n, h, w, cout), dtype=torch.float32, device=x.device)
+    covered = cin == 64 and cmid == 128 and cout == 128 and w <= 48
+    mid = None if covered else torch.empty((n, h, w, cmid), dtype=torch.float32, device=x.device)
+    _lib.check(_lib.lib().hsefr_pwblk_f16split(x.data_ptr(), img2.data_ptr(), ds2.data_ptr(), shift2.data_ptr(), w_hwc.data_ptr(), dscale.data_ptr(),
+                                               dshift.data_ptr(), img3.data_ptr(), ds3.data_ptr(), shift3.data_ptr(),
+                                               None if mid is None else mid.data_ptr(), y.data_ptr(), n, h, w, cin, cmid, cout, a_log2, a_log2_blk,
+                                               act, segs, _lib.current_stream_ptr()), "hsefr_pwblk_f16split")
     return y
 
 
diff --git a/include/hsefr.h b/include/hsefr.h
--- a/include/hsefr.h
+++ b/include/hsefr.h
@@ -89,7 +89,8 @@
     HSEFR_OPF_PAIR_NEXT = 1,
     HSEFR_OPF_HEADS = 2,
     HSEFR_OPF_OUT_SUB2 = 4,
-    HSEFR_OPF_DWPW_NEXT = 8
+    HSEFR_OPF_DWPW_NEXT = 8,
+    HSEFR_OPF_PWBLK_NEXT = 16
 } hsefr_op_flags;
 
 enum {
@@ -210,6 +211,10 @@
                         const float* descale, const float* pshift, float* y, int n, int h, int w, int c, int stride,
                         int pad_t, int pad_l, int oh, int ow, int cout, int a_log2, int act, hsefr_stream_t stream);
 
+int hsefr_pwblk_f16split(const float* x, const void* w2_split, const float* descale2, const float* shift2, const float* wd, const float* dscale,
+                         const float* dshift, const void* w3_split, const float* descale3, const float* shift3, float* mid, float* y, int n, int h,
+                         int w, int cin, int cmid, int cout, int a_log2, int a_log2_blk, int act, int segs, hsefr_stream_t stream);
+
 int hsefr_stem2_fused(const float* x, const float* conv_w, const float* conv_shift, const float* wd1, const float* d1scale,
                       const float* d1shift, const void* w_split, const float* descale, const float* pshift, const float* wd2,
                       const float* d2scale, const float* d2shift, float* y, int n, int h, int w, int cpad_t, int cpad_l,
```

Result: faster. 258,700 (median of 6 runs) (+5.1%).
